# pcannon67/pocketkaldi

Measured on AMD Instinct MI355X. Metric: acoustic frames/sec (fbank->nnet log-likelihoods), higher is better.
Workload: dtype f32

## Files before the change

### pocketkaldi_amd/csrc/capi_batch.hip

```cpp
#include <hip/hip_runtime.h>

#include <algorithm>
#include <mutex>
#include <unordered_set>
#include <vector>

#include "pk_frontend.h"
#include "pk_resample.h"
#include "pk_score.h"

using namespace pkmi;
using namespace pkhost;

namespace pkhost {
struct ArenaRec {
  void *mem;
  bool batch_alive;
  ViewGen *cur;
};
}

namespace {
std::mutex g_arena_mu;
std::unordered_set<const ViewGen *> g_gens;
std::vector<ViewGen *> g_retired;
size_t g_retired_head = 0;

inline unsigned SerialOf(const pk_mi355_am_t *am) { return (unsigned)((reinterpret_cast<uintptr_t>(am) >> 1) & 31u); }
inline pk_mi355_am_t *TagView(ViewGen *g) { return reinterpret_cast<pk_mi355_am_t *>(reinterpret_cast<uintptr_t>(g) | (uintptr_t(g->serial) << 1) | 1u); }
ViewGen *NewGenRecord(pk_mi355_am_t *am, ArenaRec *a, int views) {
  ViewGen *v;
  if (g_retired.size() - g_retired_head >= 64) {
    v = g_retired[g_retired_head++];
    if (g_retired_head > 4096) { g_retired.erase(g_retired.begin(), g_retired.begin() + g_retired_head); g_retired_head = 0; }
  } else {
    v = new ViewGen();
    v->serial = 0;
  }
  v->am = am; v->arena = a; v->live = views; v->current = true; v->withheld = false;
  g_gens.insert(v);
  return v;
}
void RetireGenRecord(ViewGen *v) {
  g_gens.erase(v);
  v->serial = (v->serial + 1) & 31u;
  g_retired.push_back(v);
}
ArenaRec *RegisterArena(void *p) { return new ArenaRec{p, true, nullptr}; }
pk_mi355_am_t *NewViewGen(ArenaRec *a, pk_mi355_am_t *am, int views) {
  std::lock_guard<std::mutex> g(g_arena_mu);
  if (a->cur) {
    a->cur->current = false;
    if (a->cur->live <= 0) RetireGenRecord(a->cur);
  }
  a->cur = NewGenRecord(am, a, views);
  return TagView(a->cur);
}
void RetireArena(ArenaRec *a) {
  void *release = nullptr;
  {
    std::lock_guard<std::mutex> g(g_arena_mu);
    a->batch_alive = false;
    if (!a->cur || a->cur->live <= 0) {
      if (a->cur) RetireGenRecord(a->cur);
      release = a->mem;
      delete a;
    }
  }
  if (release) hipHostFree(release);
}
}

namespace pkhost {
void ReleaseArenaView(pk_mi355_am_t *handle) {
  void *release = nullptr;
  {
    std::lock_guard<std::mutex> g(g_arena_mu);
    ViewGen *v = GenOf(handle);
    if (!g_gens.count(v) || v->serial != SerialOf(handle)) return;
    if (--v->live > 0) return;
    if (v->current) {
      ArenaRec *a = v->arena;
      if (a->batch_alive) return;
      release = a->mem;
      delete a;
    }
    RetireGenRecord(v);
  }
  if (release) hipHostFree(release);
}
}

namespace {
hipStream_t ResultStream(int device) {
  static hipStream_t streams[64] = {};
  if (device < 0 || device >= 64) { Fail(PK_MI355_E_INVALID, "device index %d", device); return nullptr; }
  std::lock_guard<std::mutex> g(g_arena_mu);
  if (!streams[device]) {
    hipError_t e = hipStreamCreateWithFlags(&streams[device], hipStreamNonBlocking);
    if (e != hipSuccess) { Fail(PK_MI355_E_DEVICE, "result stream: %s", hipGetErrorString(e)); return nullptr; }
  }
  return streams[device];
}
}


struct pk_mi355_batch {
  ScorerCore core;
  Timer timer;
  int max_utts = 0;
  int64_t max_samples = 0;
  float *d_wave = nullptr;
  int16_t *d_wave_i16 = nullptr;
  const float *wave_f32 = nullptr;
  const int16_t *wave_i16 = nullptr;
  enum Source { kNone, kWaves, kRaw, kNormalized };
  Source source = kNone;
  bool features_only = false;
  bool have_stats = false;
  FrontendAnyTables *d_any = nullptr;
  float *d_feats = nullptr;
  const float *feats = nullptr;
  Resampler resampler;
  float *h_native = nullptr, *d_native = nullptr;
  int64_t native_cap = 0;
  int num_utts = 0;
  int max_T = 0;
  int64_t total_frames = 0, total_cols = 0;
  int64_t dirty_cols = 0;
  char *h_lay = nullptr, *d_lay = nullptr;
  hipEvent_t ev_layout = nullptr;
  int64_t *h_wave_off = nullptr, *h_raw_base = nullptr, *h_pad_base = nullptr;
  int32_t *h_T = nullptr;
  UttLayout lay{};
  std::vector<int64_t> h_out_base;
  int64_t total_rows = 0;
  bool compact = false;
  const int32_t *d_shift4 = nullptr;
  float *d_raw_alloc = nullptr;
  float *d_raw = nullptr;
  _Float16 *d_y2 = nullptr;
  float *h_ll = nullptr;
  ArenaRec *arena = nullptr;
  hipEvent_t ev_scored = nullptr, ev_fetched = nullptr;
  int lanes = 1;
  hipStream_t stream2 = nullptr;
  ExecBufs exec2;
  hipEvent_t ev_front = nullptr, ev_lane2 = nullptr;
  bool scored = false;
  bool range_pending = false;
  int range_status = 0;
  char range_msg[512] = "";
};

namespace {

constexpr size_t kLayoutEntry = 3 * sizeof(int64_t) + sizeof(int32_t);

int FramesFit(const pk_mi355_batch *b, const int *frames, int num_utts) {
  const int pad = b->core.am->left + b->core.am->right;
  int64_t raw = 0, col = 0;
  for (int u = 0; u < num_utts; ++u) {
    raw += frames[u];
    col += frames[u] > 0 ? frames[u] + pad : 0;
  }
  if (raw > b->core.max_frames || RoundUp(col, kTile) > b->core.max_cols)
    return Fail(PK_MI355_E_INVALID, "frame capacity exceeded (%lld frames, %lld columns; the batch holds %lld and %lld)", (long long)raw,
                (long long)RoundUp(col, kTile), (long long)b->core.max_frames, (long long)b->core.max_cols);
  return 0;
}

int SetLayoutFrames(pk_mi355_batch *b, const int *frames, const int *num_samples, int num_utts) {
  if (int rc = FramesFit(b, frames, num_utts)) return rc;
  ScorerCore &c = b->core;
  const int pad = c.am->left + c.am->right;
  HIP_TRY(hipEventSynchronize(b->ev_layout));
  const size_t n = (size_t)num_utts;
  size_t bytes = kLayoutEntry * n;
  b->h_wave_off = reinterpret_cast<int64_t *>(b->h_lay); b->h_raw_base = b->h_wave_off + n; b->h_pad_base = b->h_raw_base + n;
  b->h_T = reinterpret_cast<int32_t *>(b->h_pad_base + n);
  const int64_t *d64 = reinterpret_cast<const int64_t *>(b->d_lay);
  b->lay = UttLayout{d64, reinterpret_cast<const int32_t *>(d64 + 3 * n), d64 + n, d64 + 2 * n};
  int64_t woff = 0, raw = 0, col = 0;
  b->max_T = 0;
  for (int u = 0; u < num_utts; ++u) {
    const int T = frames[u];
    b->h_wave_off[u] = woff; b->h_raw_base[u] = raw; b->h_pad_base[u] = col; b->h_T[u] = T;
    woff += num_samples ? num_samples[u] : 0;
    raw += T;
    col += T > 0 ? T + pad : 0;
    b->max_T = std::max(b->max_T, T);
  }
  if (col < b->dirty_cols)
    HIP_TRY(hipMemset2DAsync(c.d_yt + col, sizeof(float) * c.ldy, 0, sizeof(float) * (size_t)(b->dirty_cols - col), c.am->feat_dim, c.stream));
  b->dirty_cols = col;
  b->num_utts = num_utts;
  b->total_frames = raw;
  b->total_cols = col;
  b->scored = false;
  b->h_out_base.resize(num_utts);
  b->total_rows = 0;
  int64_t row = 0;
  std::vector<ShiftSpan> spans;
  bool shifted = false;
  for (int u = 0; u < num_utts; ++u) {
    const int T = b->h_T[u];
    b->h_out_base[u] = b->compact ? row : b->h_pad_base[u];
    if (T == 0) continue;
    b->total_rows = b->h_out_base[u] + T;
    row += RoundUp(T, 4);
    spans.push_back({row, (int32_t)(b->h_pad_base[u] - b->h_out_base[u])});
    shifted = shifted || spans.back().shift != 0;
  }
  b->d_shift4 = nullptr;
  if (num_utts == 0) return 0;
  if (shifted) {
    bytes = RoundUp(bytes, 256);
    if (!ExpandShift4(spans, b->total_rows, c.zero_span, reinterpret_cast<int32_t *>(b->h_lay + bytes), nullptr))
      return Fail(PK_MI355_E_INVALID, "internal: column shift outside [0, %lld]", (long long)(c.zero_span - kTile));
    b->d_shift4 = reinterpret_cast<const int32_t *>(b->d_lay + bytes);
    bytes += sizeof(int32_t) * Shift4Groups(b->total_rows);
  }
  HIP_TRY(hipMemcpyAsync(b->d_lay, b->h_lay, bytes, hipMemcpyHostToDevice, c.stream));
  HIP_TRY(hipEventRecord(b->ev_layout, c.stream));
  return 0;
}

int SetLayout(pk_mi355_batch *b, const int *num_samples, int num_utts) {
  if (num_utts < 0 || num_utts > b->max_utts) return Fail(PK_MI355_E_INVALID, "too many utterances (%d > %d)", num_utts, b->max_utts);
  std::vector<int> frames(num_utts);
  int64_t total = 0;
  for (int u = 0; u < num_utts; ++u) {
    if (num_samples[u] < 0) return Fail(PK_MI355_E_INVALID, "negative sample count");
    frames[u] = pk_mi355_num_frames(num_samples[u]);
    total += num_samples[u];
  }
  if (total > b->max_samples) return Fail(PK_MI355_E_INVALID, "too many samples (%lld > %lld)", (long long)total, (long long)b->max_samples);
  if (int rc = SetLayoutFrames(b, frames.data(), num_samples, num_utts)) return rc;
  b->source = pk_mi355_batch::kWaves;
  return 0;
}

int CheckFeatureKind(const pk_mi355_batch *b, int kind) {
  if (kind != PK_MI355_FEATS_NORMALIZED && kind != PK_MI355_FEATS_RAW) return Fail(PK_MI355_E_INVALID, "unknown feature kind %d", kind);
  if (kind == PK_MI355_FEATS_RAW && !b->have_stats) {
    if (b->core.am->feat_dim == kNumBins)
      return Fail(PK_MI355_E_INVALID, "raw features need the CMVN statistics and a %d-dim model (this batch: no statistics, %d-dim)", kNumBins,
                  kNumBins);
    return Fail(PK_MI355_E_INVALID, "raw features need the CMVN statistics: this %d-dim batch was made without them "
                "(pk_mi355_features_batch_create_stats takes the %d of a %d-dim model)", b->core.am->feat_dim, b->core.am->feat_dim + 1,
                b->core.am->feat_dim);
  }
  return 0;
}
int CheckFeatureCounts(const pk_mi355_batch *b, const int *frames, int num_utts) {
  if (num_utts < 0 || num_utts > b->max_utts) return Fail(PK_MI355_E_INVALID, "too many utterances (%d > %d)", num_utts, b->max_utts);
  for (int u = 0; u < num_utts; ++u)
    if (frames[u] < 0) return Fail(PK_MI355_E_INVALID, "utterance %d has a negative frame count (%d)", u, frames[u]);
  return FramesFit(b, frames, num_utts);
}
int EnsureFeatsStaging(pk_mi355_batch *b) {
  if (b->d_feats) return 0;
  HIP_TRY(hipMalloc(&b->d_feats, sizeof(float) * (size_t)b->core.max_frames * b->core.am->feat_dim));
  return 0;
}
int WaveEntryAllowed(const pk_mi355_batch *b) {
  if (b->features_only) return Fail(PK_MI355_E_STATE, "this batch was made by pk_mi355_features_batch_create: it takes features, not audio");
  return 0;
}

int BatchRangeStatus(pk_mi355_batch *b) {
  if (b->range_pending) {
    const ExecBufs *eb[2] = {&b->core.exec, &b->exec2};
    b->range_status = EvalRange(b->core.am, eb, b->lanes == 2 ? 2 : 1);
    if (b->range_status) {
      snprintf(b->range_msg, sizeof(b->range_msg), "%s", LastError());
      std::lock_guard<std::mutex> g(g_arena_mu);
      if (b->arena && b->arena->cur) b->arena->cur->withheld = true;
    }
    b->range_pending = false;
  }
  if (b->range_status) return Fail(b->range_status, "%s", b->range_msg);
  return 0;
}

int64_t TotalSamples(const int *num_samples, int n) {
  int64_t s = 0;
  for (int i = 0; i < n; ++i) s += num_samples[i];
  return s;
}

}

namespace pkhost {
bool BatchScored(const pk_mi355_batch *b) { return b->scored; }
const pk_mi355_am *BatchModel(const pk_mi355_batch *b) { return b->core.am; }

void CreateScorerCore(ScorerCore *c, pk_mi355_am *am, const float *global_stats, int stats_dim, int units, int64_t max_frames,
                      int64_t max_rows, int64_t chunk_cap, CreateCheck &chk) {
  const int pad = am->left + am->right;
  c->am = am; c->device = am->device; c->max_frames = max_frames;
  c->max_cols = RoundUp(max_rows + (int64_t)units * pad, kTileF16);
  c->chunk = std::min<int64_t>(chunk_cap, c->max_cols);
  c->zero_span = ZeroSpan(units, pad);
  c->ldy = RoundUp(c->max_cols, c->chunk) + 256 + c->zero_span;
  auto table = [&](auto **d, const void *h, size_t bytes) {
    chk(hipMalloc(d, bytes));
    if (chk.ok) chk(hipMemcpy(*d, h, bytes, hipMemcpyHostToDevice));
  };
  chk(hipStreamCreate(&c->stream));
  if (global_stats) {
    if (stats_dim == kNumBins) {
      FrontendTables host;
      if (BuildFrontendTables(&host)) { chk.ok = false; Fail(PK_MI355_E_INVALID, "front-end table construction failed"); }
      table(&c->d_tables, &host, sizeof(FrontendTables));
    }
    CmvnTables ctab;
    BuildCmvnTables(global_stats[stats_dim], &ctab);
    table(&c->d_global, global_stats, sizeof(float) * (stats_dim + 1));
    table(&c->d_cmvn_tab, &ctab, sizeof(CmvnTables));
  }
  chk(hipMalloc(&c->d_yt, sizeof(float) * c->ldy * am->feat_dim));
  if (chk.ok) chk(hipMemset(c->d_yt, 0, sizeof(float) * c->ldy * am->feat_dim));
  chk(hipMalloc(&c->d_ll, sizeof(float) * c->max_cols * am->num_pdfs));
  if (chk.ok && AllocExec(am, c->chunk, &c->exec)) chk.ok = false;
}

void FreeScorerCore(ScorerCore *c) {
  FreeExec(&c->exec);
  hipFree(c->d_tables); hipFree(c->d_global); hipFree(c->d_cmvn_tab); hipFree(c->d_yt); hipFree(c->d_ll);
  if (c->stream) hipStreamDestroy(c->stream);
}

bool ExpandShift4(const std::vector<ShiftSpan> &spans, int64_t total_rows, int64_t zero_span, int32_t *shift4, int32_t *bad) {
  int32_t shift = 0;
  int64_t g = 0;
  for (const ShiftSpan &sp : spans) {
    shift = sp.shift;
    if (shift < 0 || shift + kTile > zero_span) { if (bad) *bad = shift; return false; }
    for (; g < sp.end_row / 4; ++g) shift4[g] = shift;
  }
  for (const int64_t groups = Shift4Groups(total_rows); g < groups; ++g) shift4[g] = shift;
  return true;
}
}

extern "C" {

int pk_mi355_num_frames(int num_samples) {
  if (num_samples < kFrameLength) return 0;
  return 1 + (num_samples - kFrameLength) / kFrameShift;
}

}

namespace {
int64_t PublicChunkCap() {
  const char *e = getenv("PK_MI355_CHUNK");
  return e && atol(e) >= kTile ? RoundUp(atol(e), kTileF16) : 262144;
}

pk_mi355_batch *CreateBatch(pk_mi355_am_t *am, const float *global_stats, int max_utts, int64_t max_total_samples, int64_t max_frames,
                            int64_t chunk_cap, const FrontendAnyTables *any = nullptr) {
  if (UseDevice(am->device)) return nullptr;
  pk_mi355_batch *b = new pk_mi355_batch();
  ScorerCore &c = b->core;
  b->max_utts = max_utts; b->max_samples = max_total_samples;
  b->features_only = max_total_samples == 0;
  b->have_stats = global_stats != nullptr;
  const int pad = am->left + am->right;
  CreateCheck chk{b->features_only ? "batch_create_features" : "batch_create"};
  CreateScorerCore(&c, am, global_stats, am->feat_dim, max_utts, max_frames, max_frames, chunk_cap, chk);
  b->compact = pad >= 3;
  if (const char *e = getenv("PK_MI355_COMPACT_ROWS")) b->compact = b->compact && atoi(e) != 0;
  const size_t lay_bytes = RoundUp(kLayoutEntry * max_utts, 256) + (b->compact ? sizeof(int32_t) * Shift4Cap(c.max_cols) : 0);
  chk(hipHostMalloc(reinterpret_cast<void **>(&b->h_lay), lay_bytes, hipHostMallocDefault));
  chk(hipMalloc(&b->d_lay, lay_bytes));
  chk(hipEventCreateWithFlags(&b->ev_layout, hipEventDisableTiming));
  if (b->have_stats && am->feat_dim != kNumBins) {
    chk(hipMalloc(&b->d_raw_alloc, sizeof(float) * (size_t)c.max_frames * am->feat_dim));
    b->d_raw = b->d_raw_alloc;
  } else if (b->have_stats) {
    const size_t raw_floats = (size_t)c.max_frames * kNumBins + kCmvnRawLead + kCmvnRawSlack;
    chk(hipMalloc(&b->d_raw_alloc, sizeof(float) * raw_floats));
    if (chk.ok) chk(hipMemset(b->d_raw_alloc, 0, sizeof(float) * raw_floats));
    if (chk.ok) b->d_raw = b->d_raw_alloc + kCmvnRawLead;
  }
  if (any) {
    if (!c.d_tables && chk.ok) {
      FrontendTables host;
      if (BuildFrontendTables(&host)) { chk.ok = false; Fail(PK_MI355_E_INVALID, "front-end table construction failed"); }
      chk(hipMalloc(&c.d_tables, sizeof(FrontendTables)));
      if (chk.ok) chk(hipMemcpy(c.d_tables, &host, sizeof(FrontendTables), hipMemcpyHostToDevice));
    }
    chk(hipMalloc(&b->d_any, sizeof(FrontendAnyTables)));
    if (chk.ok) chk(hipMemcpy(b->d_any, any, sizeof(FrontendAnyTables), hipMemcpyHostToDevice));
    if (am->feat_dim != kNumBins)
      chk(hipMalloc(&b->d_feats, sizeof(float) * (size_t)c.max_frames * am->feat_dim));
  }
  if (IsF16(am->precision)) chk(hipMalloc(&b->d_y2, sizeof(_Float16) * 2 * c.ldy * am->feat_dim));
  if (const char *e = getenv("PK_MI355_LANES")) b->lanes = atoi(e) >= 2 ? 2 : 1;
  if (c.max_cols <= c.chunk) b->lanes = 1;
  if (b->lanes == 2) {
    chk(hipStreamCreate(&b->stream2));
    chk(hipEventCreateWithFlags(&b->ev_front, hipEventDisableTiming));
    chk(hipEventCreateWithFlags(&b->ev_lane2, hipEventDisableTiming));
    if (chk.ok && AllocExec(am, c.chunk, &b->exec2)) chk.ok = false;
  }
  if (!chk.ok) { pk_mi355_batch_destroy(b); return nullptr; }
  return b;
}

template <class Make>
pk_mi355_batch *EnsureOwned(OwnedBatch *o, int64_t need, bool keep, Make make) {
  if (o->b && need <= o->cap && keep) return o->b;
  if (o->b) pk_mi355_batch_destroy(o->b);
  o->cap = std::max<int64_t>(need, 2 * o->cap);
  o->b = make(o->cap);
  if (!o->b) o->cap = 0;
  return o->b;
}
}

namespace pkhost {
pk_mi355_batch *SingleBatch(pk_mi355_am *am, int64_t frames) {
  return EnsureOwned(&am->single, std::max(frames, kSingleChunk), true,
                     [&](int64_t cap) { return CreateBatch(am, nullptr, 1, 0, cap, kSingleChunk); });
}
}

extern "C" {

pk_mi355_batch_t *pk_mi355_batch_create(pk_mi355_am_t *am, const float *global_stats41, int max_utts, int64_t max_total_samples) {
  if (!am || !am->finalized) { Fail(PK_MI355_E_STATE, "model not finalized"); return nullptr; }
  if (am->feat_dim != kNumBins) { Fail(PK_MI355_E_INVALID, "the front-end produces %d-dim features, the model expects %d", kNumBins, am->feat_dim); return nullptr; }
  if (!global_stats41 || max_utts <= 0 || max_total_samples <= 0) { Fail(PK_MI355_E_INVALID, "bad batch capacity"); return nullptr; }
  return CreateBatch(am, global_stats41, max_utts, max_total_samples, max_total_samples / kFrameShift + max_utts, PublicChunkCap());
}

pk_mi355_batch_t *pk_mi355_features_batch_create(pk_mi355_am_t *am, const float *global_stats41, int max_utts, int64_t max_total_frames) {
  if (!am || !am->finalized) { Fail(PK_MI355_E_STATE, "model not finalized"); return nullptr; }
  if (max_utts <= 0 || max_total_frames <= 0) { Fail(PK_MI355_E_INVALID, "bad batch capacity"); return nullptr; }
  if (global_stats41 && am->feat_dim != kNumBins) {
    Fail(PK_MI355_E_INVALID, "the CMVN statistics are for %d-dim features, the model expects %d", kNumBins, am->feat_dim);
    return nullptr;
  }
  if (IsF16(am->precision) && am->feat_dim % 8 != 0) {
    Fail(PK_MI355_E_INVALID, "f16x3 / f16 precision needs a feature dimension that is a multiple of 8 (got %d)", am->feat_dim);
    return nullptr;
  }
  return CreateBatch(am, global_stats41, max_utts, 0, max_total_frames, PublicChunkCap());
}

pk_mi355_batch_t *pk_mi355_features_batch_create_stats(pk_mi355_am_t *am, const float *global_stats, int stats_len, int max_utts,
                                                       int64_t max_total_frames) {
  if (!am || !am->finalized) { Fail(PK_MI355_E_STATE, "model not finalized"); return nullptr; }
  if (!global_stats) { Fail(PK_MI355_E_INVALID, "null argument"); return nullptr; }
  if (stats_len != am->feat_dim + 1) {
    Fail(PK_MI355_E_INVALID, "the CMVN statistics have %d entries, a %d-dim model needs %d (the sums, then the count)", stats_len, am->feat_dim,
         am->feat_dim + 1);
    return nullptr;
  }
  if (am->feat_dim == kNumBins) return pk_mi355_features_batch_create(am, global_stats, max_utts, max_total_frames);
  if (max_utts <= 0 || max_total_frames <= 0) { Fail(PK_MI355_E_INVALID, "bad batch capacity"); return nullptr; }
  if (IsF16(am->precision) && am->feat_dim % 8 != 0) {
    Fail(PK_MI355_E_INVALID, "f16x3 / f16 precision needs a feature dimension that is a multiple of 8 (got %d)", am->feat_dim);
    return nullptr;
  }
  return CreateBatch(am, global_stats, max_utts, 0, max_total_frames, PublicChunkCap());
}

pk_mi355_batch_t *pk_mi355_frontend_batch_create(pk_mi355_am_t *am, const pk_mi355_frontend_spec_t *spec, const float *global_stats,
                                                 int stats_len, int max_utts, int64_t max_total_samples) {
  if (!am || !am->finalized) { Fail(PK_MI355_E_STATE, "model not finalized"); return nullptr; }
  if (!spec || !global_stats) { Fail(PK_MI355_E_INVALID, "null argument"); return nullptr; }
  std::vector<FrontendAnyTables> any(1);
  if (BuildFrontendAnyTables(spec, any.data())) return nullptr;
  if (any[0].dim != am->feat_dim) {
    Fail(PK_MI355_E_INVALID, "the front-end spec produces %d-dim features, the model expects %d", any[0].dim, am->feat_dim);
    return nullptr;
  }
  if (stats_len != am->feat_dim + 1) {
    Fail(PK_MI355_E_INVALID, "the CMVN statistics have %d entries, a %d-dim model needs %d (the sums, then the count)", stats_len, am->feat_dim,
         am->feat_dim + 1);
    return nullptr;
  }
  if (max_utts <= 0 || max_total_samples <= 0) { Fail(PK_MI355_E_INVALID, "bad batch capacity"); return nullptr; }
  if (IsF16(am->precision) && am->feat_dim % 8 != 0) {
    Fail(PK_MI355_E_INVALID, "f16x3 / f16 precision needs a feature dimension that is a multiple of 8 (got %d)", am->feat_dim);
    return nullptr;
  }
  return CreateBatch(am, global_stats, max_utts, max_total_samples, max_total_samples / kFrameShift + max_utts, PublicChunkCap(), any.data());
}

int pk_mi355_features_dim(const pk_mi355_batch_t *b) { return b ? b->core.am->feat_dim : 0; }

void pk_mi355_batch_destroy(pk_mi355_batch_t *b) {
  if (!b) return;
  hipSetDevice(b->core.device);
  if (b->core.stream) hipStreamSynchronize(b->core.stream);
  if (b->stream2) hipStreamSynchronize(b->stream2);
  FreeExec(&b->exec2);
  for (hipEvent_t e : {b->ev_front, b->ev_lane2, b->ev_scored, b->ev_fetched, b->ev_layout}) if (e) hipEventDestroy(e);
  if (b->stream2) hipStreamDestroy(b->stream2);
  hipFree(b->d_wave); hipFree(b->d_wave_i16); hipFree(b->d_raw_alloc); hipFree(b->d_y2); hipFree(b->d_feats); hipFree(b->d_any);
  b->resampler.Free();
  if (b->h_native) hipHostFree(b->h_native);
  hipFree(b->d_native);
  if (b->h_lay) hipHostFree(b->h_lay);
  hipFree(b->d_lay);
  if (b->arena) RetireArena(b->arena);
  FreeScorerCore(&b->core);
  delete b;
}

int pk_mi355_batch_set_waves(pk_mi355_batch_t *b, const pk_vector_t *waves, int num_utts) {
  if (!b || !waves) return Fail(PK_MI355_E_INVALID, "null argument");
  if (int rc = WaveEntryAllowed(b)) return rc;
  if (int rc = UseDevice(b->core.device)) return rc;
  std::vector<int> ns(num_utts);
  for (int u = 0; u < num_utts; ++u) ns[u] = waves[u].dim;
  if (TotalSamples(ns.data(), num_utts) > b->max_samples) return Fail(PK_MI355_E_INVALID, "too many samples");
  if (!b->d_wave) HIP_TRY(hipMalloc(&b->d_wave, sizeof(float) * b->max_samples));
  int64_t off = 0;
  for (int u = 0; u < num_utts; ++u) {
    if (ns[u] > 0)
      HIP_TRY(hipMemcpyAsync(b->d_wave + off, waves[u].data, sizeof(float) * ns[u], hipMemcpyHostToDevice, b->core.stream));
    off += ns[u];
  }
  b->wave_f32 = b->d_wave;
  b->wave_i16 = nullptr;
  return SetLayout(b, ns.data(), num_utts);
}

int pk_mi355_resample_set_waves(pk_mi355_batch_t *b, const pk_vector_t *waves, const int *rates, int num_utts) {
  if (!b || !waves) return Fail(PK_MI355_E_INVALID, "null argument");
  if (int rc = WaveEntryAllowed(b)) return rc;
  bool native = false;
  for (int u = 0; rates && u < num_utts; ++u) native = native || rates[u] != kSampleRate;
  if (!native) return pk_mi355_batch_set_waves(b, waves, num_utts);
  if (num_utts > b->max_utts) return Fail(PK_MI355_E_INVALID, "too many utterances (%d > %d)", num_utts, b->max_utts);
  if (int rc = UseDevice(b->core.device)) return rc;
  std::vector<int> ns(num_utts);
  std::vector<const DeviceResampleTable *> tab(num_utts, nullptr);
  int64_t total_native = 0;
  for (int u = 0; u < num_utts; ++u) {
    if (waves[u].dim < 0) return Fail(PK_MI355_E_INVALID, "negative sample count");
    if (rates[u] == kSampleRate) { ns[u] = waves[u].dim; continue; }
    if (int rc = b->resampler.Table(rates[u], &tab[u])) return rc;
    const int64_t n_out = ResampleNumOutput(tab[u]->host, waves[u].dim);
    if (n_out > b->max_samples) return Fail(PK_MI355_E_INVALID, "too many samples");
    ns[u] = (int)n_out;
    total_native += waves[u].dim;
  }
  if (TotalSamples(ns.data(), num_utts) > b->max_samples) return Fail(PK_MI355_E_INVALID, "too many samples");
  if (!b->d_wave) HIP_TRY(hipMalloc(&b->d_wave, sizeof(float) * b->max_samples));
  HIP_TRY(hipStreamSynchronize(b->core.stream));
  if (total_native > b->native_cap) {
    const int64_t cap = std::max<int64_t>(total_native, 2 * b->native_cap);
    if (b->h_native) hipHostFree(b->h_native);
    hipFree(b->d_native);
    b->h_native = nullptr; b->d_native = nullptr; b->native_cap = 0;
    HIP_TRY(hipHostMalloc(reinterpret_cast<void **>(&b->h_native), sizeof(float) * cap, hipHostMallocDefault));
    HIP_TRY(hipMalloc(&b->d_native, sizeof(float) * cap));
    b->native_cap = cap;
  }
  std::vector<ResampleItem> items;
  int64_t off = 0, noff = 0;
  for (int u = 0; u < num_utts; ++u) {
    const int n = waves[u].dim;
    if (!tab[u]) {
      if (n > 0) HIP_TRY(hipMemcpyAsync(b->d_wave + off, waves[u].data, sizeof(float) * n, hipMemcpyHostToDevice, b->core.stream));
    } else {
      if (n > 0) memcpy(b->h_native + noff, waves[u].data, sizeof(float) * n);
      if (ns[u] > 0) items.push_back(Resampler::Item(*tab[u], b->d_native + noff, 0, n, 0, ns[u], b->d_wave + off));
      noff += n;
    }
    off += ns[u];
  }
  if (total_native > 0)
    HIP_TRY(hipMemcpyAsync(b->d_native, b->h_native, sizeof(float) * total_native, hipMemcpyHostToDevice, b->core.stream));
  if (int rc = b->resampler.Run(items, b->core.stream)) return rc;
  b->wave_f32 = b->d_wave;
  b->wave_i16 = nullptr;
  return SetLayout(b, ns.data(), num_utts);
}

int pk_mi355_batch_set_waves_i16(pk_mi355_batch_t *b, const int16_t *samples, const int *num_samples,
                                 int num_utts) {
  if (!b || !samples || !num_samples) return Fail(PK_MI355_E_INVALID, "null argument");
  if (int rc = WaveEntryAllowed(b)) return rc;
  if (int rc = UseDevice(b->core.device)) return rc;
  const int64_t total = TotalSamples(num_samples, num_utts);
  if (total > b->max_samples) return Fail(PK_MI355_E_INVALID, "too many samples");
  if (!b->d_wave_i16) HIP_TRY(hipMalloc(&b->d_wave_i16, sizeof(int16_t) * b->max_samples));
  if (total > 0)
    HIP_TRY(hipMemcpyAsync(b->d_wave_i16, samples, sizeof(int16_t) * total, hipMemcpyHostToDevice, b->core.stream));
  b->wave_i16 = b->d_wave_i16;
  b->wave_f32 = nullptr;
  return SetLayout(b, num_samples, num_utts);
}

int pk_mi355_batch_set_waves_device(pk_mi355_batch_t *b, const float *d_samples, const int *num_samples,
                                    int num_utts) {
  if (!b || !d_samples || !num_samples) return Fail(PK_MI355_E_INVALID, "null argument");
  if (int rc = WaveEntryAllowed(b)) return rc;
  if (int rc = UseDevice(b->core.device)) return rc;
  b->wave_f32 = d_samples;
  b->wave_i16 = nullptr;
  return SetLayout(b, num_samples, num_utts);
}

int pk_mi355_features_set(pk_mi355_batch_t *b, const pk_matrix_t *feats, int num_utts, int kind) {
  if (!b || (num_utts > 0 && !feats)) return Fail(PK_MI355_E_INVALID, "null argument");
  if (int rc = CheckFeatureKind(b, kind)) return rc;
  const int D = b->core.am->feat_dim;
  std::vector<int> frames(std::max(num_utts, 0));
  for (int u = 0; u < num_utts; ++u) {
    if (feats[u].nrow != D) return Fail(PK_MI355_E_INVALID, "features of utterance %d have %d rows, the model expects %d", u, feats[u].nrow, D);
    if (feats[u].ncol > 0 && !feats[u].data) return Fail(PK_MI355_E_INVALID, "features of utterance %d: null data", u);
    frames[u] = feats[u].ncol;
  }
  if (int rc = CheckFeatureCounts(b, frames.data(), num_utts)) return rc;
  if (int rc = UseDevice(b->core.device)) return rc;
  float *dst = b->d_raw;
  if (kind == PK_MI355_FEATS_NORMALIZED || D != kNumBins)
    if (int rc = EnsureFeatsStaging(b)) return rc;
  if (kind == PK_MI355_FEATS_NORMALIZED) dst = b->d_feats;
  if (int rc = SetLayoutFrames(b, frames.data(), nullptr, num_utts)) return rc;
  b->source = pk_mi355_batch::kNone;
  int64_t row = 0;
  for (int u = 0; u < num_utts; ++u) {
    if (frames[u] > 0)
      HIP_TRY(hipMemcpyAsync(dst + row * D, feats[u].data, sizeof(float) * (size_t)frames[u] * D, hipMemcpyHostToDevice, b->core.stream));
    row += frames[u];
  }
  if (kind == PK_MI355_FEATS_NORMALIZED) b->feats = b->d_feats;
  b->source = kind == PK_MI355_FEATS_RAW ? pk_mi355_batch::kRaw : pk_mi355_batch::kNormalized;
  return 0;
}

int pk_mi355_features_set_device(pk_mi355_batch_t *b, const float *d_feats, const int *num_frames, int num_utts, int kind) {
  if (!b || (num_utts > 0 && (!d_feats || !num_frames))) return Fail(PK_MI355_E_INVALID, "null argument");
  if (int rc = CheckFeatureKind(b, kind)) return rc;
  if (int rc = CheckFeatureCounts(b, num_frames, num_utts)) return rc;
  if (int rc = UseDevice(b->core.device)) return rc;
  if (kind == PK_MI355_FEATS_RAW) {
    const int D = b->core.am->feat_dim;
    if (D != kNumBins)
      if (int rc = EnsureFeatsStaging(b)) return rc;
    int64_t total = 0;
    for (int u = 0; u < num_utts; ++u) total += num_frames[u];
    if (total > 0)
      HIP_TRY(hipMemcpyAsync(b->d_raw, d_feats, sizeof(float) * (size_t)total * D, hipMemcpyDeviceToDevice, b->core.stream));
  }
  if (int rc = SetLayoutFrames(b, num_frames, nullptr, num_utts)) return rc;
  if (kind == PK_MI355_FEATS_NORMALIZED) b->feats = d_feats;
  b->source = kind == PK_MI355_FEATS_RAW ? pk_mi355_batch::kRaw : pk_mi355_batch::kNormalized;
  return 0;
}

int pk_mi355_batch_score(pk_mi355_batch_t *b, float prob_scale, int sync) {
  if (!b) return Fail(PK_MI355_E_INVALID, "null batch");
  if (b->source == pk_mi355_batch::kNone) return Fail(PK_MI355_E_STATE, "no waves or features set");
  ScorerCore &c = b->core;
  int rc = UseDevice(c.device);
  if (rc) return rc;
  pk_mi355_am *am = c.am;
  Timer *tm = b->timer.enabled ? &b->timer : nullptr;
  if (tm) tm->Reset();
  b->range_pending = false;
  b->range_status = 0;
  b->range_msg[0] = 0;
  b->scored = false;
  if (b->num_utts == 0 || b->total_frames == 0) { b->scored = true; return 0; }
  const UttLayout &lay = b->lay;
  const int D = am->feat_dim;
  if (b->source == pk_mi355_batch::kWaves) {
    Scoped t(tm, PK_MI355_K_FBANK, c.stream);
    if (b->d_any) LaunchFbankAny(b->wave_f32, b->wave_i16, lay, b->num_utts, b->max_T, c.d_tables, b->d_any, D, b->d_raw, c.stream);
    else LaunchFbank(b->wave_f32, b->wave_i16, lay, b->num_utts, b->max_T, c.d_tables, b->d_raw, c.stream);
  }
  {
    Scoped t(tm, PK_MI355_K_CMVN, c.stream);
    if (b->source == pk_mi355_batch::kNormalized)
      LaunchFeatureLayout(b->feats, lay, b->num_utts, b->max_T, D, am->left, am->right, c.d_yt, c.ldy, c.stream);
    else if (D != kNumBins) {
      LaunchCmvnChain(b->d_raw, lay, b->num_utts, D, c.d_global, c.d_cmvn_tab, b->d_feats, c.stream);
      LaunchFeatureLayout(b->d_feats, lay, b->num_utts, b->max_T, D, am->left, am->right, c.d_yt, c.ldy, c.stream);
    } else
      LaunchCmvn(b->d_raw, lay, b->num_utts, c.d_global, c.d_cmvn_tab, am->left, am->right, c.d_yt, c.ldy, c.stream);
  }
  const bool f16 = IsF16(am->precision);
  if (f16) {
    if ((rc = BeginRange(c.exec, c.stream))) return rc;
    Scoped t(tm, PK_MI355_K_OTHER, c.stream);
    const int split_rows = (int)std::min<int64_t>(c.ldy, RoundUp(b->total_cols, kTileF16) + 2 * kTileF16);
    LaunchSplitF16(c.d_yt, 1, c.ldy, split_rows, D, D, b->d_y2, 2 * D, ExpX(am, 0), RangeOf(c.exec, 0), c.stream);
  }
  const bool two = b->lanes == 2 && b->total_rows > c.chunk;
  if (f16 && b->lanes == 2 && !two) ClearHostRange(b->exec2);
  if (two) {
    HIP_TRY(hipEventRecord(b->ev_front, c.stream));
    HIP_TRY(hipStreamWaitEvent(b->stream2, b->ev_front, 0));
    if (f16 && (rc = BeginRange(b->exec2, b->stream2))) return rc;
  }
  const Operand op{c.d_yt, b->d_y2, c.ldy, ZeroSource(c), b->d_shift4};
  const Lane lanes[2] = {{c.stream, &c.exec}, {b->stream2, &b->exec2}};
  if ((rc = WalkChunks(am, op, b->total_rows, c.chunk, lanes, two ? 2 : 1, true, prob_scale, c.d_ll, tm))) return rc;
  if (two) {
    if (f16 && (rc = CollectRange(b->exec2, b->stream2))) return rc;
    HIP_TRY(hipEventRecord(b->ev_lane2, b->stream2));
    HIP_TRY(hipStreamWaitEvent(c.stream, b->ev_lane2, 0));
  }
  if (f16) {
    if ((rc = CollectRange(c.exec, c.stream))) return rc;
    b->range_pending = true;
    b->range_status = 0;
  }
  b->scored = true;
  if (sync) return pk_mi355_batch_synchronize(b);
  return 0;
}

int pk_mi355_batch_synchronize(pk_mi355_batch_t *b) {
  if (!b) return Fail(PK_MI355_E_INVALID, "null batch");
  HIP_TRY(hipStreamSynchronize(b->core.stream));
  return BatchRangeStatus(b);
}

int pk_mi355_batch_calibrate(pk_mi355_batch_t *b) {
  if (!b) return Fail(PK_MI355_E_INVALID, "null batch");
  pk_mi355_am *am = b->core.am;
  if (!IsF16(am->precision)) return 0;
  if (b->source == pk_mi355_batch::kNone) return Fail(PK_MI355_E_STATE, "no waves or features set");
  if (b->total_frames == 0) return Fail(PK_MI355_E_INVALID, "calibration needs at least one frame");
  if (int rc = UseDevice(b->core.device)) return rc;
  std::lock_guard<std::mutex> lock(am->mu);
  return BatchCalibrateLocked(b);
}

}

int pkhost::BatchCalibrateLocked(pk_mi355_batch *b) {
  pk_mi355_am *am = b->core.am;
  if (am->exps_stale) if (int rc = RefreshExps(am)) return rc;
  const ExecBufs &e = b->core.exec;
  return CalibrateLoop(am, e, [&]() -> int {
    const int rc = pk_mi355_batch_score(b, 1.0f, 0);
    b->scored = false;
    b->range_pending = false;
    if (rc) return rc;
    HIP_TRY(hipStreamSynchronize(b->core.stream));
    if (b->lanes == 2)
      for (int i = 0; i < e.range_words; ++i) e.h_range[i] = std::max(e.h_range[i], b->exec2.h_range[i]);
    return 0;
  });
}

extern "C" {

int pk_mi355_batch_num_utts(const pk_mi355_batch_t *b) { return b ? b->num_utts : 0; }
int pk_mi355_batch_num_frames(const pk_mi355_batch_t *b, int utt) {
  return (b && utt >= 0 && utt < b->num_utts) ? b->h_T[utt] : 0;
}
int64_t pk_mi355_batch_total_frames(const pk_mi355_batch_t *b) { return b ? b->total_frames : 0; }

const float *pk_mi355_batch_loglik_device(const pk_mi355_batch_t *b, int utt) {
  if (!b || utt < 0 || utt >= b->num_utts) return nullptr;
  return b->core.d_ll + b->h_out_base[utt] * b->core.am->num_pdfs;
}

int pk_mi355_batch_fetch(pk_mi355_batch_t *b, int utt, pk_decodable_t *out) {
  if (!b || !out || utt < 0 || utt >= b->num_utts) return Fail(PK_MI355_E_INVALID, "bad utterance index");
  if (!b->scored) return Fail(PK_MI355_E_STATE, "batch not scored");
  if (int rc = UseDevice(b->core.device)) return rc;
  ClearDecodable(out, b->core.am);
  if (b->h_T[utt] == 0) return 0;
  return FetchRows(pk_mi355_batch_loglik_device(b, utt), b->h_T[utt], b->core.am->num_pdfs, b->core.stream, "fetch", out,
                   [&] { return BatchRangeStatus(b); });
}

int pk_mi355_batch_fetch_all(pk_mi355_batch_t *b, pk_decodable_t *out, int num_out, int sync) {
  if (!b || !out || num_out != b->num_utts) return Fail(PK_MI355_E_INVALID, "fetch_all: expected %d decodables", b ? b->num_utts : 0);
  if (!b->scored) return Fail(PK_MI355_E_STATE, "batch not scored");
  int rc = UseDevice(b->core.device);
  if (rc) return rc;
  const int N = b->core.am->num_pdfs;
  if (!b->h_ll) {
    const size_t bytes = sizeof(float) * (size_t)b->core.max_cols * N;
    HIP_TRY(hipHostMalloc(reinterpret_cast<void **>(&b->h_ll), bytes, hipHostMallocDefault));
    b->arena = RegisterArena(b->h_ll);
  }
  if (b->total_rows > 0) {
    hipStream_t rs = ResultStream(b->core.device);
    if (!rs) return PK_MI355_E_DEVICE;
    if (!b->ev_scored) {
      HIP_TRY(hipEventCreateWithFlags(&b->ev_scored, hipEventDisableTiming));
      HIP_TRY(hipEventCreateWithFlags(&b->ev_fetched, hipEventDisableTiming));
    }
    HIP_TRY(hipEventRecord(b->ev_scored, b->core.stream));
    HIP_TRY(hipStreamWaitEvent(rs, b->ev_scored, 0));
    HIP_TRY(hipMemcpyAsync(b->h_ll, b->core.d_ll, sizeof(float) * (size_t)b->total_rows * N, hipMemcpyDeviceToHost, rs));
    HIP_TRY(hipEventRecord(b->ev_fetched, rs));
    HIP_TRY(hipStreamWaitEvent(b->core.stream, b->ev_fetched, 0));
  }
  pk_mi355_am_t *gen = NewViewGen(b->arena, b->core.am, num_out);
  for (int u = 0; u < num_out; ++u) {
    const int T = b->h_T[u];
    out[u].am = gen;
    out[u].log_prob.ncol = T;
    out[u].log_prob.nrow = T > 0 ? N : 0;
    out[u].log_prob.data = T > 0 ? b->h_ll + (size_t)b->h_out_base[u] * N : nullptr;
  }
  if (sync && (rc = pk_mi355_batch_synchronize(b))) {
    for (int u = 0; u < num_out; ++u) {
      ReleaseArenaView(gen);
      ClearDecodable(&out[u], b->core.am);
    }
    return rc;
  }
  return 0;
}

int pk_mi355_batch_fetch_fbank(pk_mi355_batch_t *b, int utt, float *out) {
  if (!b || !out || utt < 0 || utt >= b->num_utts) return Fail(PK_MI355_E_INVALID, "bad utterance index");
  if (!b->scored) return Fail(PK_MI355_E_STATE, "batch not scored");
  if (b->source == pk_mi355_batch::kNormalized) return Fail(PK_MI355_E_STATE, "the batch was fed normalised features: there is no fbank");
  const int T = b->h_T[utt];
  if (T == 0) return 0;
  const int D = b->core.am->feat_dim;
  HIP_TRY(hipMemcpyAsync(out, b->d_raw + b->h_raw_base[utt] * D, sizeof(float) * (size_t)T * D, hipMemcpyDeviceToHost, b->core.stream));
  HIP_TRY(hipStreamSynchronize(b->core.stream));
  return 0;
}

int pk_mi355_batch_fetch_cmvn(pk_mi355_batch_t *b, int utt, float *out) {
  if (!b || !out || utt < 0 || utt >= b->num_utts) return Fail(PK_MI355_E_INVALID, "bad utterance index");
  if (!b->scored) return Fail(PK_MI355_E_STATE, "batch not scored");
  const int T = b->h_T[utt];
  if (T == 0) return 0;
  const int D = b->core.am->feat_dim;
  std::vector<float> tmp((size_t)D * T);
  HIP_TRY(hipMemcpy2DAsync(tmp.data(), sizeof(float) * T, b->core.d_yt + b->h_pad_base[utt] + b->core.am->left,
                           sizeof(float) * b->core.ldy, sizeof(float) * T, D, hipMemcpyDeviceToHost, b->core.stream));
  HIP_TRY(hipStreamSynchronize(b->core.stream));
  for (int t = 0; t < T; ++t)
    for (int d = 0; d < D; ++d) out[(size_t)t * D + d] = tmp[(size_t)d * T + t];
  return 0;
}

int pk_mi355_batch_gather_loglik(pk_mi355_batch_t *b, int utt, const int32_t *d_frames,
                                 const int32_t *d_trans_ids, int n, float *d_out) {
  if (!b || utt < 0 || utt >= b->num_utts || !d_frames || !d_trans_ids || !d_out)
    return Fail(PK_MI355_E_INVALID, "bad gather arguments");
  if (!b->scored) return Fail(PK_MI355_E_STATE, "batch not scored");
  if (int rc = UseDevice(b->core.device)) return rc;
  LaunchGather(pk_mi355_batch_loglik_device(b, utt), b->core.am->num_pdfs, b->core.am->d_tid2pdf,
               (int)b->core.am->tid2pdf.size(), d_frames, d_trans_ids, n, d_out, b->core.stream);
  hipError_t e = hipGetLastError();
  if (e != hipSuccess) return Fail(PK_MI355_E_DEVICE, "gather: %s", hipGetErrorString(e));
  return 0;
}

void *pk_mi355_batch_stream(pk_mi355_batch_t *b) { return b ? (void *)b->core.stream : nullptr; }

int pk_mi355_batch_enable_timing(pk_mi355_batch_t *b, int enable) {
  if (!b) return Fail(PK_MI355_E_INVALID, "null batch");
  b->timer.enabled = enable != 0;
  if (!enable) b->timer.Reset();
  return 0;
}

int pk_mi355_batch_get_timing(pk_mi355_batch_t *b, float ms[PK_MI355_K_COUNT], int launches[PK_MI355_K_COUNT]) {
  if (!b) return Fail(PK_MI355_E_INVALID, "null batch");
  for (int k = 0; k < PK_MI355_K_COUNT; ++k) { ms[k] = 0; launches[k] = 0; }
  HIP_TRY(hipStreamSynchronize(b->core.stream));
  for (auto &r : b->timer.recs) {
    float t = 0;
    HIP_TRY(hipEventElapsedTime(&t, r.a, r.b));
    ms[r.kind] += t;
    launches[r.kind] += 1;
  }
  return 0;
}

int pk_mi355_process_acoustic(pk_mi355_am_t *am, const pk_vector_t *cmvn_global_stats,
                              const pk_vector_t *raw_wave, float prob_scale, pk_decodable_t *out,
                              int verbose) {
  if (!am || !cmvn_global_stats || !raw_wave || !out) return Fail(PK_MI355_E_INVALID, "null argument");
  if (cmvn_global_stats->dim != kNumBins + 1) return Fail(PK_MI355_E_INVALID, "cmvn_global_stats must have 41 entries");
  ClearDecodable(out, am);
  if (raw_wave->dim == 0) return 0;
  std::lock_guard<std::mutex> lock(am->mu);
  const float *stats = cmvn_global_stats->data;
  pk_mi355_batch *b = EnsureOwned(&am->proc, std::max<int64_t>(raw_wave->dim, 16000), memcmp(am->proc_stats, stats, sizeof(am->proc_stats)) == 0,
                                  [&](int64_t cap) { return pk_mi355_batch_create(am, stats, 1, cap); });
  if (!b) return PK_MI355_E_DEVICE;
  memcpy(am->proc_stats, stats, sizeof(am->proc_stats));
  int rc = pk_mi355_batch_set_waves(b, raw_wave, 1);
  if (rc) return rc;
  pk_mi355_batch_enable_timing(b, verbose);
  if ((rc = pk_mi355_batch_score(b, prob_scale, 1))) return rc;
  if (verbose) {
    float ms[PK_MI355_K_COUNT];
    int launches[PK_MI355_K_COUNT];
    if ((rc = pk_mi355_batch_get_timing(b, ms, launches))) return rc;
    fprintf(stderr, "Fbank: %lfms\n", (double)ms[PK_MI355_K_FBANK]);
    fprintf(stderr, "CMVN: %lfms\n", (double)ms[PK_MI355_K_CMVN]);
    fprintf(stderr, "NNET: %lfms\n", (double)(ms[PK_MI355_K_GEMM] + ms[PK_MI355_K_TAIL] + ms[PK_MI355_K_OTHER]));
  }
  return pk_mi355_batch_fetch(b, 0, out);
}

}
```

### pocketkaldi_amd/csrc/capi_exec.hip

```cpp
#include <hip/hip_runtime.h>
#include <math.h>

#include <algorithm>
#include <mutex>
#include <vector>

#include "pk_score.h"

using namespace pkmi;
using namespace pkhost;

namespace pkhost {

struct ExecResult { const float *data = nullptr; int64_t ld = 0; int dim = 0; };

int AllocExec(const pk_mi355_am *am, int64_t rows_cap, ExecBufs *e) {
  e->rows_cap = rows_cap;
  if (IsF16(am->precision)) {
    const size_t act = sizeof(_Float16) * 2 * (size_t)am->max_dim_pad * rows_cap;
    const size_t xin = sizeof(_Float16) * 2 * (size_t)RoundUp(am->input_dim, kBKF16) * (rows_cap + 16);
    for (int i = 0; i < 2; ++i) {
      HIP_TRY(hipMalloc(&e->h[i], act));
      HIP_TRY(hipMemset(e->h[i], 0, act));
    }
    HIP_TRY(hipMalloc(&e->xin, xin));
    HIP_TRY(hipMemset(e->xin, 0, xin));
    e->range_words = (int)am->lin.size() * kRangeSlots;
    HIP_TRY(hipMalloc(&e->range, sizeof(uint32_t) * e->range_words));
    HIP_TRY(hipMemset(e->range, 0, sizeof(uint32_t) * e->range_words));
    HIP_TRY(hipHostMalloc(reinterpret_cast<void **>(&e->h_range), sizeof(uint32_t) * e->range_words, hipHostMallocDefault));
    memset(e->h_range, 0, sizeof(uint32_t) * e->range_words);
  }
  {
    const size_t nd = sizeof(unsigned) * (size_t)(rows_cap / kTile + 2);
    HIP_TRY(hipMalloc(&e->row_done, nd));
    HIP_TRY(hipMemset(e->row_done, 0, nd));
    e->row_done_bytes = nd;
  }
  e->act_floats = (int64_t)am->max_dim_pad * rows_cap;
  e->in_floats = RoundUp(am->input_dim, kBK) * rows_cap;
  HIP_TRY(hipMalloc(&e->a, e->act_floats * sizeof(float)));
  HIP_TRY(hipMalloc(&e->b, e->act_floats * sizeof(float)));
  HIP_TRY(hipMalloc(&e->in, e->in_floats * sizeof(float)));
  HIP_TRY(hipMemset(e->a, 0, e->act_floats * sizeof(float)));
  HIP_TRY(hipMemset(e->b, 0, e->act_floats * sizeof(float)));
  HIP_TRY(hipMemset(e->in, 0, e->in_floats * sizeof(float)));
  return 0;
}

void FreeExec(ExecBufs *e) {
  hipFree(e->a);
  hipFree(e->b);
  hipFree(e->in);
  for (int i = 0; i < 2; ++i) hipFree(e->h[i]);
  hipFree(e->xin);
  hipFree(e->range);
  hipFree(e->row_done);
  if (e->h_range) hipHostFree(e->h_range);
  *e = ExecBufs();
}

int BeginRange(const ExecBufs &e, hipStream_t s) {
  if (e.range) HIP_TRY(hipMemsetAsync(e.range, 0, sizeof(uint32_t) * e.range_words, s));
  return 0;
}
int CollectRange(const ExecBufs &e, hipStream_t s) {
  if (e.range) HIP_TRY(hipMemcpyAsync(e.h_range, e.range, sizeof(uint32_t) * e.range_words, hipMemcpyDeviceToHost, s));
  return 0;
}
void ClearHostRange(const ExecBufs &e) {
  if (e.h_range) memset(e.h_range, 0, sizeof(uint32_t) * e.range_words);
}
float RangeMax(const ExecBufs &e, int l) {
  uint32_t m = 0;
  for (int i = 0; i < kRangeSlots; ++i) m = std::max(m, e.h_range[(size_t)l * kRangeSlots + i]);
  float f;
  memcpy(&f, &m, sizeof(f));
  return f;
}
int EvalRange(const pk_mi355_am *am, const ExecBufs *const *bufs, int nbufs) {
  const int nlin = (int)am->lin.size();
  for (int l = 0; l < nlin; ++l) {
    float m = 0.0f;
    for (int i = 0; i < nbufs; ++i)
      if (bufs[i]->h_range) m = std::max(m, RangeMax(*bufs[i], l));
    const int xe = am->exps_stale ? 0 : am->h_exps[nlin + l];
    const char *mode = am->precision == PK_MI355_PRECISION_F16 ? "f16" : "f16x3";
    if (m >= kRangeSaturated)
      return Fail(PK_MI355_E_RANGE, "%s range: the input of affine layer %d saturated (|x| * 2^%d reached 65504, the fp16 split "
                  "clamps there): results withheld; lower the operand's exponent (pk_mi355_am_calibrate)", mode, l, xe);
    if (m > 0.0f && m < kRangeTooSmall)
      return Fail(PK_MI355_E_RANGE, "%s range: the input of affine layer %d is too small for the fp16 split (max |x| * 2^%d = %g "
                  "< 2^-5: every low half is subnormal): results withheld; raise the operand's exponent "
                  "(pk_mi355_am_calibrate)", mode, l, xe, (double)m);
  }
  return 0;
}


int RunLayers(const pk_mi355_am *am, const ExecBufs &e, const float *q0, int64_t ldq,
              int splice_dim, int rows, bool want_tail, float scale, float *tail_out,
              int64_t tail_ld, hipStream_t stream, Timer *timer, ExecResult *res, const float *splice_zero = nullptr,
              const int32_t *splice_shift = nullptr) {
  const int rows_pad = (int)RoundUp(rows, kTile);
  if (splice_dim > 0 && !splice_zero) return Fail(PK_MI355_E_INVALID, "spliced input without a zero source");
  if (rows_pad > e.rows_cap) return Fail(PK_MI355_E_INVALID, "chunk larger than workspace");
  const float *blob = am->d_blob;
  const int nl = (int)am->layers.size();

  int last_linear = -1;
  for (int i = 0; i < nl; ++i)
    if (am->layers[i].type == PK_NNET_LINEAR_LAYER) last_linear = i;

  const float *cur = splice_dim > 0 ? q0 : e.in;
  int64_t cur_ld = splice_dim > 0 ? ldq : e.rows_cap;
  bool cur_rows = false;
  bool cur_splice = splice_dim > 0;
  int cur_dim = am->input_dim;
  float *bufs[2] = {e.a, e.b};
  int next_buf = 0;
  int li_lin = 0;
  bool tail_done = false;

  auto to_rows = [&]() {
    float *dst = bufs[next_buf];
    const int64_t ld = RoundUp(cur_dim, kTile);
    Scoped t(timer, PK_MI355_K_OTHER, stream);
    LaunchTransposeToRows(cur, cur_ld, cur_dim, rows_pad, dst, ld, stream);
    cur = dst; cur_ld = ld; cur_rows = true; next_buf ^= 1;
  };

  for (int i = 0; i < nl; ++i) {
    const HostLayer &L = am->layers[i];
    switch (L.type) {
      case PK_NNET_LINEAR_LAYER: {
        const DevLinear &D = am->lin[li_lin++];
        if (cur_rows) return Fail(PK_MI355_E_INVALID, "linear layer after a softmax is not supported");
        const bool fuse_relu = (i + 1 < nl && am->layers[i + 1].type == PK_NNET_RELU_LAYER);
        const bool rows_out = (i == last_linear) && !cur_splice;
        float *dst = bufs[next_buf];
        GemmArgs g;
        g.K = D.Kpad;
        g.relu = fuse_relu ? 1 : 0;
        g.bias = blob + D.b_off;
        g.out = dst;
        if (!rows_out) {
          g.P = blob + D.wt_off; g.ldp = D.Npad;
          g.Q = cur; g.ldq = cur_ld;
          g.splice_dim = cur_splice ? splice_dim : 0;
          if (cur_splice) {
            g.splice_ctx = am->left + am->right + 1;
            g.splice_zero = splice_zero;
            g.splice_shift = splice_shift;
            g.ring = am->knobs.l1_ring;
          }
          g.bias_on_j = 0;
          g.ldo = e.rows_cap;
          g.tiles_i = D.Npad / kTile; g.tiles_j = rows_pad / kTile;
        } else {
          g.P = cur; g.ldp = cur_ld;
          g.Q = blob + D.wt_off; g.ldq = D.Npad;
          g.splice_dim = 0;
          g.bias_on_j = 1;
          g.ldo = D.Npad;
          g.tiles_i = rows_pad / kTile; g.tiles_j = D.Npad / kTile;
        }
        bool fused_tail = false;
        if (rows_out && want_tail && !fuse_relu && !am->softmax_reference && i + 2 == nl &&
            am->layers[i + 1].type == PK_NNET_SOFTMAX_LAYER && am->knobs.wave_tail32) {
          g.tail_out = tail_out; g.tail_ld = tail_ld;
          g.tail_log_prior = blob + am->logprior_off; g.tail_scale = scale;
          g.tail_n = D.N; g.tail_rows = rows; g.row_done = e.row_done;
          g.tail_walk = am->knobs.tail_walk;
          fused_tail = GemmFusesTail(g, am->knobs.fused_tail_min_tiles);
          if (!fused_tail) g.tail_out = nullptr;
          else HIP_TRY(hipMemsetAsync(e.row_done, 0, sizeof(unsigned) * (size_t)g.tiles_i, stream));
        }
        {
          Scoped t(timer, PK_MI355_K_GEMM, stream);
          GemmArgs fewer = g;
          fewer.tiles_j -= 1;
          if (fused_tail && am->knobs.tail_strip && g.tiles_j > 8 && D.N <= (g.tiles_j - 1) * kTile + kTile / 2 &&
              GemmFusesTail(fewer, am->knobs.fused_tail_min_tiles)) {
            GemmArgs s = g;
            const int j0 = (g.tiles_j - 1) * kTile;
            s.Q = g.Q + j0; s.bias = g.bias + j0; s.out = g.out + j0;
            s.half_j = 1;
            s.tail_out = nullptr;
            LaunchGemm(s, stream);
            g.tiles_j -= 1;
          }
          LaunchGemm(g, stream);
        }
        cur = dst; cur_ld = g.ldo; cur_rows = rows_out; cur_splice = false; cur_dim = D.N;
        next_buf ^= 1;
        if (fuse_relu) ++i;
        if (fused_tail) { tail_done = true; ++i; }
        break;
      }
      case PK_NNET_RELU_LAYER: {
        if (cur_splice || cur == e.in) {
          float *dst = bufs[next_buf];
          if (cur_splice) return Fail(PK_MI355_E_INVALID, "network must start with a linear layer when splicing");
          HIP_TRY(hipMemcpyAsync(dst, cur, sizeof(float) * (size_t)RoundUp(cur_dim, kBK) * e.rows_cap,
                                 hipMemcpyDeviceToDevice, stream));
          cur = dst; next_buf ^= 1;
        }
        Scoped t(timer, PK_MI355_K_OTHER, stream);
        const int64_t n = cur_rows ? (int64_t)rows_pad * cur_ld : (int64_t)cur_dim * cur_ld;
        LaunchRelu(const_cast<float *>(cur), n, stream);
        break;
      }
      case PK_NNET_NORMALIZE_LAYER: {
        if (cur_splice) return Fail(PK_MI355_E_INVALID, "network must start with a linear layer when splicing");
        if (cur == e.in) {
          float *dst = bufs[next_buf];
          HIP_TRY(hipMemcpyAsync(dst, cur, sizeof(float) * (size_t)RoundUp(cur_dim, kBK) * e.rows_cap,
                                 hipMemcpyDeviceToDevice, stream));
          cur = dst; next_buf ^= 1;
        }
        Scoped t(timer, PK_MI355_K_OTHER, stream);
        if (cur_rows) LaunchNormalize(const_cast<float *>(cur), rows_pad, cur_dim, cur_ld, 1, stream);
        else LaunchNormalize(const_cast<float *>(cur), rows_pad, cur_dim, 1, cur_ld, stream);
        break;
      }
      case PK_NNET_SOFTMAX_LAYER: {
        if (cur_splice) return Fail(PK_MI355_E_INVALID, "network must start with a linear layer when splicing");
        if (!cur_rows) to_rows();
        const bool final_layer = (i == nl - 1);
        Scoped t(timer, PK_MI355_K_TAIL, stream);
        if (final_layer && want_tail) {
          if (!(am->knobs.wave_tail32 && !am->softmax_reference &&
                LaunchTailWave(cur, cur_ld, rows, cur_dim, blob + am->logprior_off, scale, tail_out, tail_ld, stream)))
            LaunchTail(kTailSoftmaxLoglik, am->softmax_reference, cur, cur_ld, rows, cur_dim,
                       blob + am->logprior_off, scale, tail_out, tail_ld, stream);
          tail_done = true;
        } else {
          float *dst = bufs[next_buf];
          const int64_t ld = RoundUp(cur_dim, kTile);
          LaunchTail(kTailSoftmaxProb, am->softmax_reference, cur, cur_ld, rows_pad, cur_dim, nullptr, 1.0f, dst, ld, stream);
          cur = dst; cur_ld = ld; next_buf ^= 1;
        }
        break;
      }
      default:
        return Fail(PK_MI355_E_INVALID, "unknown layer type %d", L.type);
    }
  }
  if (!cur_rows && !tail_done) {
    if (cur_splice) return Fail(PK_MI355_E_INVALID, "empty network");
    to_rows();
  }
  if (want_tail && !tail_done) {
    Scoped t(timer, PK_MI355_K_TAIL, stream);
    LaunchTail(kTailLoglik, am->softmax_reference, cur, cur_ld, rows, cur_dim, blob + am->logprior_off,
               scale, tail_out, tail_ld, stream);
  }
  if (res) { res->data = cur; res->ld = cur_ld; res->dim = cur_dim; }
  hipError_t le = hipGetLastError();
  if (le != hipSuccess) return Fail(PK_MI355_E_DEVICE, "kernel launch failed: %s", hipGetErrorString(le));
  return 0;
}

int RunLayersF16(const pk_mi355_am *am, const ExecBufs &e, const _Float16 *x, int64_t ldx, int rows,
                 bool want_tail, float scale, float *tail_out,
                 int64_t tail_ld, hipStream_t stream, Timer *timer, ExecResult *res, const int32_t *row_shift4 = nullptr) {
  const int rows_pad = (int)RoundUp(rows, kTileF16);
  if (rows_pad > e.rows_cap) return Fail(PK_MI355_E_INVALID, "chunk larger than workspace");
  const float *blob = am->d_blob;
  const int nl = (int)am->layers.size();
  const int nlin = (int)am->lin.size();
  int li = 0, buf = 0;
  int64_t out_ld = 0;
  for (int i = 0; i < nl; ++i) {
    if (am->layers[i].type != PK_NNET_LINEAR_LAYER) continue;
    const DevLinear &D = am->lin[li];
    const bool last = (li == nlin - 1);
    GemmF16Args g;
    g.X = x; g.ldx = ldx;
    g.row_shift4 = li == 0 ? row_shift4 : nullptr;
    g.W = reinterpret_cast<const _Float16 *>(blob + D.wt_off);
    g.ldw = 2 * D.Kpad;
    g.K = D.Kpad;
    g.bias = blob + D.b_off;
    g.relu = (i + 1 < nl && am->layers[i + 1].type == PK_NNET_RELU_LAYER) ? 1 : 0;
    const int after = i + 1 + g.relu;
    const bool norm = after < nl && am->layers[after].type == PK_NNET_NORMALIZE_LAYER;
    g.out_f32 = (last || norm) ? e.a : nullptr;
    g.out = (last || norm) ? nullptr : e.h[buf];
    g.ldo = (last || norm) ? D.Npad : 2 * D.Npad;
    g.tiles_m = rows_pad / kTileF16;
    g.tiles_n = D.Npad / kTileF16;
    g.terms = am->precision == PK_MI355_PRECISION_F16 ? 1 : 3;
    g.e_w = ExpW(am, li);
    g.e_in = ExpX(am, li);
    g.e_out = (last || norm) ? ExpZero(am) : ExpX(am, li + 1);
    g.range = (last || norm) ? nullptr : RangeOf(e, li + 1);
    {
      Scoped t(timer, PK_MI355_K_GEMM, stream);
      LaunchGemmF16(g, stream);
    }
    if (norm) {
      Scoped t(timer, PK_MI355_K_OTHER, stream);
      LaunchNormalizeSplitF16(e.a, D.Npad, rows_pad, D.N, D.Npad, e.h[buf], 2 * D.Npad, ExpX(am, li + 1), RangeOf(e, li + 1), stream);
    }
    x = e.h[buf]; ldx = 2 * D.Npad;
    out_ld = D.Npad;
    buf ^= 1;
    ++li;
  }
  const int dim = am->output_dim;
  const bool softmax_last = am->layers.back().type == PK_NNET_SOFTMAX_LAYER;
  const float *cur = e.a;
  if (want_tail) {
    Scoped t(timer, PK_MI355_K_TAIL, stream);
    LaunchTail(softmax_last ? kTailSoftmaxLoglik : kTailLoglik, am->softmax_reference, cur, out_ld, rows, dim,
               blob + am->logprior_off, scale, tail_out, tail_ld, stream);
  } else if (softmax_last) {
    Scoped t(timer, PK_MI355_K_TAIL, stream);
    LaunchTail(kTailSoftmaxProb, am->softmax_reference, cur, out_ld, rows_pad, dim, nullptr, 1.0f, e.b, out_ld, stream);
    cur = e.b;
  }
  if (res) { res->data = cur; res->ld = out_ld; res->dim = dim; }
  hipError_t le = hipGetLastError();
  if (le != hipSuccess) return Fail(PK_MI355_E_DEVICE, "kernel launch failed: %s", hipGetErrorString(le));
  return 0;
}

int WalkChunks(const pk_mi355_am *am, const Operand &op, int64_t total_rows, int64_t chunk, const Lane *lanes, int nlanes,
               bool want_tail, float scale, float *out, Timer *timer) {
  const int D = am->feat_dim, N = am->num_pdfs;
  const bool f16 = IsF16(am->precision);
  for (int64_t r0 = 0; r0 < total_rows; r0 += chunk) {
    const int rows = (int)std::min<int64_t>(chunk, total_rows - r0);
    const Lane &l = lanes[r0 / chunk % nlanes];
    const int32_t *shift4 = op.shift4 ? op.shift4 + r0 / 4 : nullptr;
    float *dst = out + r0 * N;
    const int rc = f16 ? RunLayersF16(am, *l.exec, op.y2 + r0 * 2 * D, 2 * D, rows, want_tail, scale, dst, N, l.stream, timer, nullptr, shift4)
                       : RunLayers(am, *l.exec, op.yt + r0, op.ld, D, rows, want_tail, scale, dst, N, l.stream, timer, nullptr, op.zero, shift4);
    if (rc) return rc;
  }
  return 0;
}

struct Workspace {
  ExecBufs exec;
  float *d_feats = nullptr;  int64_t feats_cap = 0;
  hipStream_t stream = nullptr;
};

int EnsureWorkspace(pk_mi355_am *am, int64_t feats_floats) {
  if (!am->ws) {
    am->ws = new Workspace();
    HIP_TRY(hipStreamCreate(&am->ws->stream));
    int rc = AllocExec(am, kSingleChunk, &am->ws->exec);
    if (rc) return rc;
  }
  Workspace *w = am->ws;
  if (feats_floats > w->feats_cap) {
    hipFree(w->d_feats);
    w->feats_cap = feats_floats;
    HIP_TRY(hipMalloc(&w->d_feats, sizeof(float) * w->feats_cap));
  }
  return 0;
}

void FreeWorkspace(Workspace *w) {
  if (!w) return;
  FreeExec(&w->exec);
  hipFree(w->d_feats);
  if (w->stream) hipStreamDestroy(w->stream);
  delete w;
}

int ResizeHostMatrix(pk_matrix_t *m, int nrow, int ncol) {
  const size_t total = (size_t)nrow * ncol;
  float *p = nullptr;
  if (total > 0) {
    p = static_cast<float *>(realloc(m->data, sizeof(float) * total));
    if (!p) return Fail(PK_MI355_E_INVALID, "out of host memory");
  } else {
    free(m->data);
  }
  m->data = p;
  m->nrow = nrow;
  m->ncol = ncol;
  return 0;
}

int CalibrateStep(pk_mi355_am *am, const ExecBufs &e, std::vector<char> *settled) {
  const int nlin = (int)am->lin.size();
  static const int target = [] { const char *t = getenv("PK_MI355_CALIB_TARGET_LOG2"); const int v = t ? atoi(t) : 3; return v >= 0 && v <= 12 ? v : 3; }();
  for (int l = 0; l < nlin; ++l) {
    const float m = RangeMax(e, l);
    int32_t &xe = am->h_exps[nlin + l];
    int want = xe;
    if (m >= kRangeSaturated) want = xe - 12;
    else if (m > 0.0f && (!(*settled)[l] || m < ldexpf(1.0f, target - 2) || m >= ldexpf(1.0f, target + 4))) { want = xe + target - ilogbf(m); (*settled)[l] = 1; }
    else (*settled)[l] = 1;
    want = std::min(kMaxXExp, std::max(-kMaxXExp, want));
    if (want != xe) { xe = want; return 1; }
  }
  return 0;
}

int CalibrateLoop(pk_mi355_am *am, const ExecBufs &e, const std::function<int()> &pass) {
  const int max_passes = 6 * (int)am->lin.size() + 8;
  std::vector<char> settled(am->lin.size(), 0);
  for (int i = 0, rc; i < max_passes; ++i) {
    if ((rc = pass())) return rc;
    if (!CalibrateStep(am, e, &settled)) {
      const ExecBufs *eb = &e;
      return EvalRange(am, &eb, 1);
    }
    if ((rc = UploadExps(am))) return rc;
  }
  return Fail(PK_MI355_E_RANGE, "calibration did not settle in %d passes", max_passes);
}

}

extern "C" {

int pk_mi355_nnet_propagate(pk_mi355_am_t *am, const pk_matrix_t *in, pk_matrix_t *out) {
  if (!am || !am->finalized) return Fail(PK_MI355_E_STATE, "model not finalized");
  if (!in || !out || in->nrow != am->input_dim)
    return Fail(PK_MI355_E_INVALID, "input has %d rows, the network expects %d", in ? in->nrow : -1, am->input_dim);
  int rc = UseDevice(am->device);
  if (rc) return rc;
  std::lock_guard<std::mutex> lock(am->mu);
  const int T = in->ncol, D = in->nrow;
  if ((rc = ResizeHostMatrix(out, am->output_dim, T))) return rc;
  if (T == 0) return 0;
  if ((rc = EnsureWorkspace(am, (int64_t)T * D))) return rc;
  Workspace *w = am->ws;
  HIP_TRY(hipMemcpyAsync(w->d_feats, in->data, sizeof(float) * (size_t)T * D, hipMemcpyHostToDevice, w->stream));
  for (int64_t r0 = 0; r0 < T; r0 += kSingleChunk) {
    const int rows = (int)std::min<int64_t>(kSingleChunk, T - r0);
    ExecResult res;
    if (IsF16(am->precision)) {
      const int kp = (int)RoundUp(D, kBKF16);
      if ((rc = BeginRange(w->exec, w->stream))) return rc;
      const int64_t rows_pad = RoundUp(rows, kTileF16);
      if (rows_pad > rows)
        HIP_TRY(hipMemsetAsync(w->exec.xin + (size_t)rows * 2 * kp, 0, sizeof(_Float16) * 2 * kp * (size_t)(rows_pad - rows), w->stream));
      LaunchSplitF16(w->d_feats + r0 * D, D, 1, rows, D, kp, w->exec.xin, 2 * kp, ExpX(am, 0), RangeOf(w->exec, 0), w->stream);
      rc = RunLayersF16(am, w->exec, w->exec.xin, 2 * kp, rows, false, 1.0f, nullptr, 0, w->stream, nullptr, &res);
      if (!rc) rc = CollectRange(w->exec, w->stream);
    } else {
      LaunchTransposeToCols(w->d_feats + r0 * D, D, rows, D, w->exec.in, w->exec.rows_cap, w->stream);
      rc = RunLayers(am, w->exec, nullptr, 0, 0, rows, false, 1.0f, nullptr, 0, w->stream, nullptr, &res);
    }
    if (rc) return rc;
    HIP_TRY(hipMemcpy2DAsync(out->data + r0 * am->output_dim, sizeof(float) * am->output_dim, res.data,
                             sizeof(float) * res.ld, sizeof(float) * am->output_dim, rows,
                             hipMemcpyDeviceToHost, w->stream));
    HIP_TRY(hipStreamSynchronize(w->stream));
    if (IsF16(am->precision)) {
      const ExecBufs *eb = &w->exec;
      if ((rc = EvalRange(am, &eb, 1))) { ResizeHostMatrix(out, 0, 0); return rc; }
    }
  }
  return 0;
}


void pk_decodable_init(pk_decodable_t *self, pk_mi355_am_t *am, float prob_scale,
                       const pk_matrix_t *feats) {
  ClearDecodable(self, am);
  if (!am || !am->finalized) { Fail(PK_MI355_E_STATE, "model not finalized"); return; }
  if (!feats || feats->nrow != am->feat_dim) {
    Fail(PK_MI355_E_INVALID, "features have %d rows, the model expects %d", feats ? feats->nrow : -1, am->feat_dim);
    return;
  }
  if (UseDevice(am->device)) return;
  const int T = feats->ncol, D = feats->nrow;
  if (T <= 0) return;
  if (IsF16(am->precision) && D % 8 != 0) {
    Fail(PK_MI355_E_INVALID, "f16x3 / f16 precision needs a feature dimension that is a multiple of 8 (got %d)", D);
    return;
  }
  std::lock_guard<std::mutex> lock(am->mu);
  pk_mi355_batch *b = SingleBatch(am, T);
  if (!b || pk_mi355_features_set(b, feats, 1, PK_MI355_FEATS_NORMALIZED) || pk_mi355_batch_score(b, prob_scale, 0)) return;
  pk_mi355_batch_fetch(b, 0, self);
}

void pk_decodable_destroy(pk_decodable_t *self) {
  if (IsView(self->am)) ReleaseArenaView(self->am);
  else free(self->log_prob.data);
  ClearDecodable(self, nullptr);
}

float pk_decodable_loglikelihood(pk_decodable_t *self, int frame, int trans_id) {
  if (IsView(self->am) && GenOf(self->am)->withheld) return NAN;
  const int pdf = pk_mi355_am_transition_to_pdf(Untag(self->am), trans_id);
  return self->log_prob.data[(size_t)frame * self->log_prob.nrow + pdf];
}

bool pk_decodable_islastframe(pk_decodable_t *self, int frame) {
  return frame == self->log_prob.ncol - 1;
}

int pk_mi355_am_calibrate(pk_mi355_am_t *am, const pk_matrix_t *feats) {
  if (!am || !am->finalized) return Fail(PK_MI355_E_STATE, "model not finalized");
  if (!IsF16(am->precision)) return 0;
  if (!feats || feats->nrow != am->feat_dim || feats->ncol <= 0 || !feats->data)
    return Fail(PK_MI355_E_INVALID, "calibration features have %d rows, the model expects %d", feats ? feats->nrow : -1, am->feat_dim);
  if (feats->nrow % 8 != 0) return Fail(PK_MI355_E_INVALID, "f16x3 / f16 precision needs a feature dimension that is a multiple of 8 (got %d)", feats->nrow);
  int rc = UseDevice(am->device);
  if (rc) return rc;
  std::lock_guard<std::mutex> lock(am->mu);
  pk_mi355_batch *b = SingleBatch(am, feats->ncol);
  if (!b) return PK_MI355_E_DEVICE;
  if ((rc = pk_mi355_features_set(b, feats, 1, PK_MI355_FEATS_NORMALIZED))) return rc;
  return BatchCalibrateLocked(b);
}

}
```

### pocketkaldi_amd/csrc/pk_host.h

```cpp
#ifndef PK_HOST_H_
#define PK_HOST_H_

#include <hip/hip_runtime.h>
#include <stdint.h>
#include <stdio.h>
#include <stdlib.h>
#include <string.h>

#include <mutex>
#include <string>
#include <vector>

#include "pk_files.h"
#include "pk_kernels.h"
#include "pk_tables.h"

namespace pkhost {

using namespace pkmi;


int CurrentDevice();
int UseDevice(int device);

#define HIP_TRY(expr)                                                                  \
  do {                                                                                 \
    hipError_t e_ = (expr);                                                            \
    if (e_ != hipSuccess)                                                              \
      return ::pkhost::Fail(PK_MI355_E_DEVICE, "%s failed: %s (%s:%d)", #expr, hipGetErrorString(e_), \
                            __FILE__, __LINE__);                                       \
  } while (0)

inline int64_t RoundUp(int64_t v, int64_t m) { return (v + m - 1) / m * m; }
inline bool IsF16(int precision) { return precision == PK_MI355_PRECISION_F16X3 || precision == PK_MI355_PRECISION_F16; }

struct ModelKnobs {
  bool wave_tail32 = true;
  int fused_tail_min_tiles = 384;
  int tail_walk = 0;
  int l1_ring = 2;
  bool tail_strip = true;
};
ModelKnobs ReadModelKnobs();


struct Timer {
  bool enabled = false;
  struct Rec { int kind; hipEvent_t a, b; };
  std::vector<Rec> recs;
  std::vector<hipEvent_t> pool;
  hipEvent_t Get() {
    if (!pool.empty()) { hipEvent_t e = pool.back(); pool.pop_back(); return e; }
    hipEvent_t e;
    hipEventCreate(&e);
    return e;
  }
  void Reset() {
    for (auto &r : recs) { pool.push_back(r.a); pool.push_back(r.b); }
    recs.clear();
  }
  int Begin(int kind, hipStream_t s) {
    if (!enabled) return -1;
    Rec r{kind, Get(), Get()};
    hipEventRecord(r.a, s);
    recs.push_back(r);
    return (int)recs.size() - 1;
  }
  void End(int id, hipStream_t s) {
    if (id >= 0) hipEventRecord(recs[id].b, s);
  }
  ~Timer() {
    Reset();
    for (auto e : pool) hipEventDestroy(e);
  }
};

struct Scoped {
  Timer *t; int id; hipStream_t s;
  Scoped(Timer *t_, int kind, hipStream_t s_) : t(t_), id(t_ ? t_->Begin(kind, s_) : -1), s(s_) {}
  ~Scoped() { if (t) t->End(id, s); }
};


struct DevLinear {
  int K = 0, N = 0, Kpad = 0, Npad = 0;
  size_t wt_off = 0, b_off = 0;
};

struct Workspace;

struct OwnedBatch { pk_mi355_batch *b = nullptr; int64_t cap = 0; };

}

struct pk_mi355_am {
  int device = 0;
  std::vector<pkhost::HostLayer> layers;
  bool finalized = false;
  int precision = PK_MI355_PRECISION_F32;
  bool softmax_reference = false;
  int left = 0, right = 0, num_pdfs = 0;
  int input_dim = 0, output_dim = 0, feat_dim = 0;
  int max_dim_pad = 0;
  std::vector<int32_t> tid2pdf;
  int32_t *d_tid2pdf = nullptr;
  std::vector<pkhost::DevLinear> lin;
  float *d_blob = nullptr;
  size_t blob_floats = 0;
  size_t logprior_off = 0;
  size_t exp_off = 0;
  std::vector<int32_t> h_exps;
  bool exps_stale = false;
  double flops_per_frame = 0;
  pkhost::ModelKnobs knobs;
  std::mutex mu;
  pkhost::Workspace *ws = nullptr;
  pkhost::OwnedBatch proc;
  pkhost::OwnedBatch single;
  float proc_stats[41] = {0};
};

namespace pkhost {

int RefreshExps(pk_mi355_am *am);
int UploadExps(pk_mi355_am *am);


struct ExecBufs {
  float *in = nullptr;
  float *a = nullptr;
  float *b = nullptr;
  int64_t rows_cap = 0;
  int64_t in_floats = 0, act_floats = 0;
  _Float16 *h[2] = {nullptr, nullptr};
  _Float16 *xin = nullptr;
  uint32_t *range = nullptr, *h_range = nullptr;
  int range_words = 0;
  unsigned *row_done = nullptr;
  size_t row_done_bytes = 0;
};

int AllocExec(const pk_mi355_am *am, int64_t rows_cap, ExecBufs *e);
void FreeExec(ExecBufs *e);

inline const int32_t *ExpBase(const pk_mi355_am *am) { return reinterpret_cast<const int32_t *>(am->d_blob + am->exp_off); }
inline const int32_t *ExpW(const pk_mi355_am *am, int l) { return ExpBase(am) + l; }
inline const int32_t *ExpX(const pk_mi355_am *am, int l) { return ExpBase(am) + am->lin.size() + l; }
inline const int32_t *ExpZero(const pk_mi355_am *am) { return ExpBase(am) + 2 * am->lin.size(); }
inline uint32_t *RangeOf(const ExecBufs &e, int l) { return e.range ? e.range + (size_t)l * kRangeSlots : nullptr; }

constexpr int kMaxXExp = 30;
constexpr float kRangeSaturated = 65504.0f;
constexpr float kRangeTooSmall = 0.03125f;

int BeginRange(const ExecBufs &e, hipStream_t s);
int CollectRange(const ExecBufs &e, hipStream_t s);
void ClearHostRange(const ExecBufs &e);
int EvalRange(const pk_mi355_am *am, const ExecBufs *const *bufs, int nbufs);
void FreeWorkspace(Workspace *w);
int ResizeHostMatrix(pk_matrix_t *m, int nrow, int ncol);


struct ArenaRec;
struct alignas(64) ViewGen {
  pk_mi355_am_t *am;
  ArenaRec *arena;
  int live;
  bool current;
  bool withheld;
  unsigned serial;
};
inline bool IsView(const pk_mi355_am_t *am) { return (reinterpret_cast<uintptr_t>(am) & 1u) != 0; }
inline ViewGen *GenOf(const pk_mi355_am_t *am) { return reinterpret_cast<ViewGen *>(reinterpret_cast<uintptr_t>(am) & ~uintptr_t(63)); }
inline pk_mi355_am_t *Untag(pk_mi355_am_t *am) { return IsView(am) ? GenOf(am)->am : am; }
void ReleaseArenaView(pk_mi355_am_t *handle);

bool BatchScored(const pk_mi355_batch *b);
const pk_mi355_am *BatchModel(const pk_mi355_batch *b);

const pk_mi355_am *StreamModel(const pk_mi355_stream *s);
int StreamSlots(const pk_mi355_stream *s);
hipStream_t StreamHipStream(const pk_mi355_stream *s);
const float *StreamLoglikBase(const pk_mi355_stream *s);
bool StreamSlotFlushed(const pk_mi355_stream *s, int slot);

bool OnlineDecoderSlotOpen(const pk_mi355_online_decoder *o, int slot);
const std::vector<int> *OnlineDecoderCommittedWords(const pk_mi355_online_decoder *o, int slot);
void OnlineDecoderTailWords(const pk_mi355_online_decoder *o, int slot, std::vector<int> *words);

struct RecognizerFiles {
  pk_mi355_fst_t *fst = nullptr;
  pk_mi355_symtab_t *symtab = nullptr;
};
int LoadRecognizerFiles(const char *config_path, RecognizerFiles *out, bool any_stats = false);
constexpr int kMaxCmvnStats = 129;
void FreeRecognizerFiles(RecognizerFiles *f);
int JoinWords(const pk_mi355_symtab_t *symtab, const int *words, int count, std::string *text);

}

#endif
```

### pocketkaldi_amd/csrc/pk_score.h

```cpp
#ifndef PK_SCORE_H_
#define PK_SCORE_H_

#include <functional>

#include "pk_host.h"

namespace pkmi {

constexpr int kTailCap = kFrameLength;

struct StreamRec {
  int32_t slot;
  int32_t tail_len;
  int32_t new_len;
  int32_t tail_par;
  int32_t n_old;
  int32_t m;
  int32_t a, b;
  int32_t closed;
  int32_t cols;
  int32_t kind;
  int32_t hist_par;
  int64_t woff;
  int64_t new_off;
  int64_t raw_base;
  int64_t col_base;
  int64_t row_off;
};

void LaunchStreamAssemble(const StreamRec *recs, int n, const float *upload, float *tails, float *wave, hipStream_t stream);
void LaunchStreamCmvn(const StreamRec *recs, int n, float *rows, const float *g, const CmvnTables *tab, float *sums,
                      float *raw_hist, float *hist, int hist_len, int left, int right, float *yt, int64_t ldy, hipStream_t stream);

void LaunchStreamRawRows(const StreamRec *recs, int n, const float *upload, float *rows, hipStream_t stream);
void LaunchStreamFeatureLayout(const StreamRec *recs, int n, int max_cols, const float *upload, float *hist, int hist_len, int dim,
                               int left, int right, float *yt, int64_t ldy, hipStream_t stream);

void LaunchFeatureLayout(const float *feats, const UttLayout &utts, int num_utts, int max_frames, int dim, int left, int right,
                         float *yt, int64_t ldy, hipStream_t stream);

void LaunchCmvnChain(const float *raw, const UttLayout &utts, int num_utts, int dim, const float *d_global, const CmvnTables *d_cmvn_tab,
                     float *out, hipStream_t stream);
void LaunchStreamCmvnChain(const StreamRec *recs, int n, int dim, float *upload, const float *g, const CmvnTables *tab, float *sums,
                           float *raw_hist, hipStream_t stream);

}

namespace pkhost {

struct ScorerCore {
  pk_mi355_am *am = nullptr; int device = 0; hipStream_t stream = nullptr;
  FrontendTables *d_tables = nullptr; float *d_global = nullptr; CmvnTables *d_cmvn_tab = nullptr;
  int64_t max_frames = 0, max_cols = 0, chunk = 0, zero_span = 0, ldy = 0;
  float *d_yt = nullptr, *d_ll = nullptr;
  ExecBufs exec;
};

inline int64_t ZeroSpan(int64_t units, int pad) { return RoundUp(units * pad + 2 * kTile, 256); }
inline const float *ZeroSource(const float *yt, int64_t ld, int64_t zero_span) { return yt + (ld - zero_span); }
inline const float *ZeroSource(const ScorerCore &c) { return ZeroSource(c.d_yt, c.ldy, c.zero_span); }

struct CreateCheck {
  const char *name; bool ok = true;
  void operator()(hipError_t e) { if (e != hipSuccess && ok) { ok = false; Fail(PK_MI355_E_DEVICE, "%s: %s", name, hipGetErrorString(e)); } }
};
void CreateScorerCore(ScorerCore *c, pk_mi355_am *am, const float *global_stats, int stats_dim, int units, int64_t max_frames,
                      int64_t max_rows, int64_t chunk_cap, CreateCheck &chk);
void FreeScorerCore(ScorerCore *c);

struct ShiftSpan { int64_t end_row; int32_t shift; };
inline int64_t Shift4Groups(int64_t total_rows) { return RoundUp(total_rows, kTileF16) / 4 + kTileF16 / 4; }
inline int64_t Shift4Cap(int64_t max_cols) { return max_cols / 4 + kTileF16; }
bool ExpandShift4(const std::vector<ShiftSpan> &spans, int64_t total_rows, int64_t zero_span, int32_t *shift4, int32_t *bad);

struct Operand { const float *yt; const _Float16 *y2; int64_t ld; const float *zero; const int32_t *shift4; };
struct Lane { hipStream_t stream; const ExecBufs *exec; };
int WalkChunks(const pk_mi355_am *am, const Operand &op, int64_t total_rows, int64_t chunk, const Lane *lanes, int nlanes,
               bool want_tail, float scale, float *out, Timer *timer);

int CalibrateLoop(pk_mi355_am *am, const ExecBufs &e, const std::function<int()> &pass);

constexpr int64_t kSingleChunk = 4096;
pk_mi355_batch *SingleBatch(pk_mi355_am *am, int64_t frames);
int BatchCalibrateLocked(pk_mi355_batch *b);

inline void ClearDecodable(pk_decodable_t *out, pk_mi355_am_t *am) { out->am = am; out->log_prob = pk_matrix_t{0, 0, nullptr}; }
template <class Verdict>
int FetchRows(const float *src, int rows, int N, hipStream_t stream, const char *what, pk_decodable_t *out, Verdict verdict) {
  const size_t bytes = sizeof(float) * (size_t)rows * N;
  float *host = static_cast<float *>(malloc(bytes));
  if (!host) return Fail(PK_MI355_E_INVALID, "out of host memory");
  hipError_t e = hipMemcpyAsync(host, src, bytes, hipMemcpyDeviceToHost, stream);
  if (e == hipSuccess) e = hipStreamSynchronize(stream);
  if (e != hipSuccess) { free(host); return Fail(PK_MI355_E_DEVICE, "%s: %s", what, hipGetErrorString(e)); }
  if (int rc = verdict()) { free(host); return rc; }
  out->log_prob = pk_matrix_t{rows, N, host};
  return 0;
}

}

#endif
```

Baseline: 10.54 million.

## Run input upload and frontend on a separate stream to overlap with scoring

Adds a dedicated input stream per batch that carries the waveform/feature upload, layout copy, fbank, CMVN and f16 split for large batches. Consumption events are recorded after the first layer reads the spliced input, so the next batch's frontend can overlap the previous batch's nnet layers. Range tracking is split per layer so the first layer's range belongs to the input stream. This adds cross-stream event bookkeeping and risks ordering bugs around shared buffers (d_yt, d_raw, layout).

Result: no change. 10.53 million (-0.1%).

```diff
diff --git a/pocketkaldi_amd/csrc/capi_batch.hip b/pocketkaldi_amd/csrc/capi_batch.hip
--- a/pocketkaldi_amd/csrc/capi_batch.hip
+++ b/pocketkaldi_amd/csrc/capi_batch.hip
@@ -146,7 +146,12 @@
   int lanes = 1;
   hipStream_t stream2 = nullptr;
   ExecBufs exec2;
-  hipEvent_t ev_front = nullptr, ev_lane2 = nullptr;
+  hipEvent_t ev_lane_go = nullptr, ev_lane2 = nullptr;
+  int in_mode = 0;
+  int64_t in_min_frames = 0;
+  hipStream_t in_stream = nullptr;
+  hipEvent_t ev_front = nullptr, ev_consumed = nullptr, ev_consumed2 = nullptr, ev_caller = nullptr;
+  bool in_dirty = false, lay_dirty = false, consumed_new = false;
   bool scored = false;
   bool range_pending = false;
   int range_status = 0;
@@ -170,7 +175,61 @@
   return 0;
 }
 
-int SetLayoutFrames(pk_mi355_batch *b, const int *frames, const int *num_samples, int num_utts) {
+bool Pipelined(const pk_mi355_batch *b, int64_t frames, bool timed) { return b->in_stream && !timed && frames >= b->in_min_frames; }
+
+int InputStream(pk_mi355_batch *b, bool pipelined, hipStream_t *s) {
+  ScorerCore &c = b->core;
+  *s = c.stream;
+  if (!b->in_stream) return 0;
+  if (pipelined) {
+    if (b->lay_dirty) {
+      HIP_TRY(hipEventRecord(b->ev_consumed, c.stream));
+      b->lay_dirty = false;
+      b->consumed_new = true;
+    }
+    if (b->consumed_new) {
+      HIP_TRY(hipStreamWaitEvent(b->in_stream, b->ev_consumed, 0));
+      if (b->lanes == 2) HIP_TRY(hipStreamWaitEvent(b->in_stream, b->ev_consumed2, 0));
+      b->consumed_new = false;
+    }
+    b->in_dirty = true;
+    *s = b->in_stream;
+  } else {
+    if (b->in_dirty) {
+      HIP_TRY(hipEventRecord(b->ev_front, b->in_stream));
+      HIP_TRY(hipStreamWaitEvent(c.stream, b->ev_front, 0));
+      b->in_dirty = false;
+    }
+    b->lay_dirty = true;
+  }
+  return 0;
+}
+int SetStream(pk_mi355_batch *b, int64_t frames, hipStream_t *s) { return InputStream(b, Pipelined(b, frames, false), s); }
+int BehindCaller(pk_mi355_batch *b, hipStream_t s) {
+  if (s == b->core.stream) return 0;
+  HIP_TRY(hipEventRecord(b->ev_caller, b->core.stream));
+  HIP_TRY(hipStreamWaitEvent(s, b->ev_caller, 0));
+  return 0;
+}
+int JoinInput(pk_mi355_batch *b) {
+  if (!b->in_dirty) return 0;
+  HIP_TRY(hipEventRecord(b->ev_front, b->in_stream));
+  HIP_TRY(hipStreamWaitEvent(b->core.stream, b->ev_front, 0));
+  b->in_dirty = false;
+  return 0;
+}
+int64_t WaveFrames(const int *num_samples, int n) {
+  int64_t f = 0;
+  for (int i = 0; i < n; ++i) f += pk_mi355_num_frames(num_samples[i]);
+  return f;
+}
+int64_t SumFrames(const int *frames, int n) {
+  int64_t f = 0;
+  for (int i = 0; i < n; ++i) f += frames[i];
+  return f;
+}
+
+int SetLayoutFrames(pk_mi355_batch *b, const int *frames, const int *num_samples, int num_utts, hipStream_t stream) {
   if (int rc = FramesFit(b, frames, num_utts)) return rc;
   ScorerCore &c = b->core;
   const int pad = c.am->left + c.am->right;
@@ -192,7 +251,7 @@
     b->max_T = std::max(b->max_T, T);
   }
   if (col < b->dirty_cols)
-    HIP_TRY(hipMemset2DAsync(c.d_yt + col, sizeof(float) * c.ldy, 0, sizeof(float) * (size_t)(b->dirty_cols - col), c.am->feat_dim, c.stream));
+    HIP_TRY(hipMemset2DAsync(c.d_yt + col, sizeof(float) * c.ldy, 0, sizeof(float) * (size_t)(b->dirty_cols - col), c.am->feat_dim, stream));
   b->dirty_cols = col;
   b->num_utts = num_utts;
   b->total_frames = raw;
@@ -221,12 +280,12 @@
     b->d_shift4 = reinterpret_cast<const int32_t *>(b->d_lay + bytes);
     bytes += sizeof(int32_t) * Shift4Groups(b->total_rows);
   }
-  HIP_TRY(hipMemcpyAsync(b->d_lay, b->h_lay, bytes, hipMemcpyHostToDevice, c.stream));
-  HIP_TRY(hipEventRecord(b->ev_layout, c.stream));
-  return 0;
-}
-
-int SetLayout(pk_mi355_batch *b, const int *num_samples, int num_utts) {
+  HIP_TRY(hipMemcpyAsync(b->d_lay, b->h_lay, bytes, hipMemcpyHostToDevice, stream));
+  HIP_TRY(hipEventRecord(b->ev_layout, stream));
+  return 0;
+}
+
+int SetLayout(pk_mi355_batch *b, const int *num_samples, int num_utts, hipStream_t stream) {
   if (num_utts < 0 || num_utts > b->max_utts) return Fail(PK_MI355_E_INVALID, "too many utterances (%d > %d)", num_utts, b->max_utts);
   std::vector<int> frames(num_utts);
   int64_t total = 0;
@@ -236,7 +295,7 @@
     total += num_samples[u];
   }
   if (total > b->max_samples) return Fail(PK_MI355_E_INVALID, "too many samples (%lld > %lld)", (long long)total, (long long)b->max_samples);
-  if (int rc = SetLayoutFrames(b, frames.data(), num_samples, num_utts)) return rc;
+  if (int rc = SetLayoutFrames(b, frames.data(), num_samples, num_utts, stream)) return rc;
   b->source = pk_mi355_batch::kWaves;
   return 0;
 }
@@ -355,13 +414,16 @@
 }
 
 namespace {
+constexpr int kInputStreamDefault = 1;
+constexpr int64_t kInputStreamMinFrames = 131072;
+
 int64_t PublicChunkCap() {
   const char *e = getenv("PK_MI355_CHUNK");
   return e && atol(e) >= kTile ? RoundUp(atol(e), kTileF16) : 262144;
 }
 
 pk_mi355_batch *CreateBatch(pk_mi355_am_t *am, const float *global_stats, int max_utts, int64_t max_total_samples, int64_t max_frames,
-                            int64_t chunk_cap, const FrontendAnyTables *any = nullptr) {
+                            int64_t chunk_cap, const FrontendAnyTables *any = nullptr, bool input_stream = true) {
   if (UseDevice(am->device)) return nullptr;
   pk_mi355_batch *b = new pk_mi355_batch();
   ScorerCore &c = b->core;
@@ -403,9 +465,20 @@
   if (c.max_cols <= c.chunk) b->lanes = 1;
   if (b->lanes == 2) {
     chk(hipStreamCreate(&b->stream2));
-    chk(hipEventCreateWithFlags(&b->ev_front, hipEventDisableTiming));
+    chk(hipEventCreateWithFlags(&b->ev_lane_go, hipEventDisableTiming));
     chk(hipEventCreateWithFlags(&b->ev_lane2, hipEventDisableTiming));
     if (chk.ok && AllocExec(am, c.chunk, &b->exec2)) chk.ok = false;
+  }
+  b->in_mode = input_stream ? kInputStreamDefault : 0;
+  b->in_min_frames = kInputStreamMinFrames;
+  if (const char *e = getenv("PK_MI355_INPUT_STREAM")) b->in_mode = input_stream ? std::min(std::max(atoi(e), 0), 2) : 0;
+  if (const char *e = getenv("PK_MI355_INPUT_STREAM_MIN_FRAMES")) b->in_min_frames = std::max<int64_t>(atoll(e), 0);
+  if (b->in_mode) {
+    int least = 0, greatest = 0;
+    chk(hipDeviceGetStreamPriorityRange(&least, &greatest));
+    if (b->in_mode == 2) chk(hipStreamCreateWithPriority(&b->in_stream, hipStreamDefault, least));
+    else chk(hipStreamCreate(&b->in_stream));
+    for (hipEvent_t *e : {&b->ev_front, &b->ev_consumed, &b->ev_consumed2, &b->ev_caller}) chk(hipEventCreateWithFlags(e, hipEventDisableTiming));
   }
   if (!chk.ok) { pk_mi355_batch_destroy(b); return nullptr; }
   return b;
@@ -425,7 +498,7 @@
 namespace pkhost {
 pk_mi355_batch *SingleBatch(pk_mi355_am *am, int64_t frames) {
   return EnsureOwned(&am->single, std::max(frames, kSingleChunk), true,
-                     [&](int64_t cap) { return CreateBatch(am, nullptr, 1, 0, cap, kSingleChunk); });
+                     [&](int64_t cap) { return CreateBatch(am, nullptr, 1, 0, cap, kSingleChunk, nullptr, false); });
 }
 }
 
@@ -500,9 +573,12 @@
   hipSetDevice(b->core.device);
   if (b->core.stream) hipStreamSynchronize(b->core.stream);
   if (b->stream2) hipStreamSynchronize(b->stream2);
+  if (b->in_stream) hipStreamSynchronize(b->in_stream);
   FreeExec(&b->exec2);
-  for (hipEvent_t e : {b->ev_front, b->ev_lane2, b->ev_scored, b->ev_fetched, b->ev_layout}) if (e) hipEventDestroy(e);
+  for (hipEvent_t e : {b->ev_lane_go, b->ev_lane2, b->ev_scored, b->ev_fetched, b->ev_layout, b->ev_front, b->ev_consumed, b->ev_consumed2, b->ev_caller})
+    if (e) hipEventDestroy(e);
   if (b->stream2) hipStreamDestroy(b->stream2);
+  if (b->in_stream) hipStreamDestroy(b->in_stream);
   hipFree(b->d_wave); hipFree(b->d_wave_i16); hipFree(b->d_raw_alloc); hipFree(b->d_y2); hipFree(b->d_feats); hipFree(b->d_any);
   b->resampler.Free();
   if (b->h_native) hipHostFree(b->h_native);
@@ -522,15 +598,17 @@
   for (int u = 0; u < num_utts; ++u) ns[u] = waves[u].dim;
   if (TotalSamples(ns.data(), num_utts) > b->max_samples) return Fail(PK_MI355_E_INVALID, "too many samples");
   if (!b->d_wave) HIP_TRY(hipMalloc(&b->d_wave, sizeof(float) * b->max_samples));
+  hipStream_t st;
+  if (int rc = SetStream(b, WaveFrames(ns.data(), num_utts), &st)) return rc;
   int64_t off = 0;
   for (int u = 0; u < num_utts; ++u) {
     if (ns[u] > 0)
-      HIP_TRY(hipMemcpyAsync(b->d_wave + off, waves[u].data, sizeof(float) * ns[u], hipMemcpyHostToDevice, b->core.stream));
+      HIP_TRY(hipMemcpyAsync(b->d_wave + off, waves[u].data, sizeof(float) * ns[u], hipMemcpyHostToDevice, st));
     off += ns[u];
   }
   b->wave_f32 = b->d_wave;
   b->wave_i16 = nullptr;
-  return SetLayout(b, ns.data(), num_utts);
+  return SetLayout(b, ns.data(), num_utts, st);
 }
 
 int pk_mi355_resample_set_waves(pk_mi355_batch_t *b, const pk_vector_t *waves, const int *rates, int num_utts) {
@@ -555,7 +633,9 @@
   }
   if (TotalSamples(ns.data(), num_utts) > b->max_samples) return Fail(PK_MI355_E_INVALID, "too many samples");
   if (!b->d_wave) HIP_TRY(hipMalloc(&b->d_wave, sizeof(float) * b->max_samples));
-  HIP_TRY(hipStreamSynchronize(b->core.stream));
+  hipStream_t st;
+  if (int rc = SetStream(b, WaveFrames(ns.data(), num_utts), &st)) return rc;
+  HIP_TRY(hipStreamSynchronize(st));
   if (total_native > b->native_cap) {
     const int64_t cap = std::max<int64_t>(total_native, 2 * b->native_cap);
     if (b->h_native) hipHostFree(b->h_native);
@@ -570,7 +650,7 @@
   for (int u = 0; u < num_utts; ++u) {
     const int n = waves[u].dim;
     if (!tab[u]) {
-      if (n > 0) HIP_TRY(hipMemcpyAsync(b->d_wave + off, waves[u].data, sizeof(float) * n, hipMemcpyHostToDevice, b->core.stream));
+      if (n > 0) HIP_TRY(hipMemcpyAsync(b->d_wave + off, waves[u].data, sizeof(float) * n, hipMemcpyHostToDevice, st));
     } else {
       if (n > 0) memcpy(b->h_native + noff, waves[u].data, sizeof(float) * n);
       if (ns[u] > 0) items.push_back(Resampler::Item(*tab[u], b->d_native + noff, 0, n, 0, ns[u], b->d_wave + off));
@@ -579,11 +659,11 @@
     off += ns[u];
   }
   if (total_native > 0)
-    HIP_TRY(hipMemcpyAsync(b->d_native, b->h_native, sizeof(float) * total_native, hipMemcpyHostToDevice, b->core.stream));
-  if (int rc = b->resampler.Run(items, b->core.stream)) return rc;
+    HIP_TRY(hipMemcpyAsync(b->d_native, b->h_native, sizeof(float) * total_native, hipMemcpyHostToDevice, st));
+  if (int rc = b->resampler.Run(items, st)) return rc;
   b->wave_f32 = b->d_wave;
   b->wave_i16 = nullptr;
-  return SetLayout(b, ns.data(), num_utts);
+  return SetLayout(b, ns.data(), num_utts, st);
 }
 
 int pk_mi355_batch_set_waves_i16(pk_mi355_batch_t *b, const int16_t *samples, const int *num_samples,
@@ -594,11 +674,13 @@
   const int64_t total = TotalSamples(num_samples, num_utts);
   if (total > b->max_samples) return Fail(PK_MI355_E_INVALID, "too many samples");
   if (!b->d_wave_i16) HIP_TRY(hipMalloc(&b->d_wave_i16, sizeof(int16_t) * b->max_samples));
+  hipStream_t st;
+  if (int rc = SetStream(b, WaveFrames(num_samples, num_utts), &st)) return rc;
   if (total > 0)
-    HIP_TRY(hipMemcpyAsync(b->d_wave_i16, samples, sizeof(int16_t) * total, hipMemcpyHostToDevice, b->core.stream));
+    HIP_TRY(hipMemcpyAsync(b->d_wave_i16, samples, sizeof(int16_t) * total, hipMemcpyHostToDevice, st));
   b->wave_i16 = b->d_wave_i16;
   b->wave_f32 = nullptr;
-  return SetLayout(b, num_samples, num_utts);
+  return SetLayout(b, num_samples, num_utts, st);
 }
 
 int pk_mi355_batch_set_waves_device(pk_mi355_batch_t *b, const float *d_samples, const int *num_samples,
@@ -606,9 +688,12 @@
   if (!b || !d_samples || !num_samples) return Fail(PK_MI355_E_INVALID, "null argument");
   if (int rc = WaveEntryAllowed(b)) return rc;
   if (int rc = UseDevice(b->core.device)) return rc;
+  hipStream_t st;
+  if (int rc = SetStream(b, WaveFrames(num_samples, num_utts), &st)) return rc;
+  if (int rc = BehindCaller(b, st)) return rc;
   b->wave_f32 = d_samples;
   b->wave_i16 = nullptr;
-  return SetLayout(b, num_samples, num_utts);
+  return SetLayout(b, num_samples, num_utts, st);
 }
 
 int pk_mi355_features_set(pk_mi355_batch_t *b, const pk_matrix_t *feats, int num_utts, int kind) {
@@ -627,12 +712,14 @@
   if (kind == PK_MI355_FEATS_NORMALIZED || D != kNumBins)
     if (int rc = EnsureFeatsStaging(b)) return rc;
   if (kind == PK_MI355_FEATS_NORMALIZED) dst = b->d_feats;
-  if (int rc = SetLayoutFrames(b, frames.data(), nullptr, num_utts)) return rc;
+  hipStream_t st;
+  if (int rc = SetStream(b, SumFrames(frames.data(), num_utts), &st)) return rc;
+  if (int rc = SetLayoutFrames(b, frames.data(), nullptr, num_utts, st)) return rc;
   b->source = pk_mi355_batch::kNone;
   int64_t row = 0;
   for (int u = 0; u < num_utts; ++u) {
     if (frames[u] > 0)
-      HIP_TRY(hipMemcpyAsync(dst + row * D, feats[u].data, sizeof(float) * (size_t)frames[u] * D, hipMemcpyHostToDevice, b->core.stream));
+      HIP_TRY(hipMemcpyAsync(dst + row * D, feats[u].data, sizeof(float) * (size_t)frames[u] * D, hipMemcpyHostToDevice, st));
     row += frames[u];
   }
   if (kind == PK_MI355_FEATS_NORMALIZED) b->feats = b->d_feats;
@@ -645,6 +732,9 @@
   if (int rc = CheckFeatureKind(b, kind)) return rc;
   if (int rc = CheckFeatureCounts(b, num_frames, num_utts)) return rc;
   if (int rc = UseDevice(b->core.device)) return rc;
+  hipStream_t st;
+  if (int rc = SetStream(b, SumFrames(num_frames, num_utts), &st)) return rc;
+  if (int rc = BehindCaller(b, st)) return rc;
   if (kind == PK_MI355_FEATS_RAW) {
     const int D = b->core.am->feat_dim;
     if (D != kNumBins)
@@ -652,9 +742,9 @@
     int64_t total = 0;
     for (int u = 0; u < num_utts; ++u) total += num_frames[u];
     if (total > 0)
-      HIP_TRY(hipMemcpyAsync(b->d_raw, d_feats, sizeof(float) * (size_t)total * D, hipMemcpyDeviceToDevice, b->core.stream));
-  }
-  if (int rc = SetLayoutFrames(b, num_frames, nullptr, num_utts)) return rc;
+      HIP_TRY(hipMemcpyAsync(b->d_raw, d_feats, sizeof(float) * (size_t)total * D, hipMemcpyDeviceToDevice, st));
+  }
+  if (int rc = SetLayoutFrames(b, num_frames, nullptr, num_utts, st)) return rc;
   if (kind == PK_MI355_FEATS_NORMALIZED) b->feats = d_feats;
   b->source = kind == PK_MI355_FEATS_RAW ? pk_mi355_batch::kRaw : pk_mi355_batch::kNormalized;
   return 0;
@@ -676,45 +766,53 @@
   if (b->num_utts == 0 || b->total_frames == 0) { b->scored = true; return 0; }
   const UttLayout &lay = b->lay;
   const int D = am->feat_dim;
+  const bool pipelined = Pipelined(b, b->total_frames, tm != nullptr);
+  hipStream_t fs;
+  if ((rc = InputStream(b, pipelined, &fs))) return rc;
   if (b->source == pk_mi355_batch::kWaves) {
-    Scoped t(tm, PK_MI355_K_FBANK, c.stream);
-    if (b->d_any) LaunchFbankAny(b->wave_f32, b->wave_i16, lay, b->num_utts, b->max_T, c.d_tables, b->d_any, D, b->d_raw, c.stream);
-    else LaunchFbank(b->wave_f32, b->wave_i16, lay, b->num_utts, b->max_T, c.d_tables, b->d_raw, c.stream);
+    Scoped t(tm, PK_MI355_K_FBANK, fs);
+    if (b->d_any) LaunchFbankAny(b->wave_f32, b->wave_i16, lay, b->num_utts, b->max_T, c.d_tables, b->d_any, D, b->d_raw, fs);
+    else LaunchFbank(b->wave_f32, b->wave_i16, lay, b->num_utts, b->max_T, c.d_tables, b->d_raw, fs);
   }
   {
-    Scoped t(tm, PK_MI355_K_CMVN, c.stream);
+    Scoped t(tm, PK_MI355_K_CMVN, fs);
     if (b->source == pk_mi355_batch::kNormalized)
-      LaunchFeatureLayout(b->feats, lay, b->num_utts, b->max_T, D, am->left, am->right, c.d_yt, c.ldy, c.stream);
+      LaunchFeatureLayout(b->feats, lay, b->num_utts, b->max_T, D, am->left, am->right, c.d_yt, c.ldy, fs);
     else if (D != kNumBins) {
-      LaunchCmvnChain(b->d_raw, lay, b->num_utts, D, c.d_global, c.d_cmvn_tab, b->d_feats, c.stream);
-      LaunchFeatureLayout(b->d_feats, lay, b->num_utts, b->max_T, D, am->left, am->right, c.d_yt, c.ldy, c.stream);
+      LaunchCmvnChain(b->d_raw, lay, b->num_utts, D, c.d_global, c.d_cmvn_tab, b->d_feats, fs);
+      LaunchFeatureLayout(b->d_feats, lay, b->num_utts, b->max_T, D, am->left, am->right, c.d_yt, c.ldy, fs);
     } else
-      LaunchCmvn(b->d_raw, lay, b->num_utts, c.d_global, c.d_cmvn_tab, am->left, am->right, c.d_yt, c.ldy, c.stream);
+      LaunchCmvn(b->d_raw, lay, b->num_utts, c.d_global, c.d_cmvn_tab, am->left, am->right, c.d_yt, c.ldy, fs);
   }
   const bool f16 = IsF16(am->precision);
+  const int first_own = f16 && b->in_stream ? 1 : 0;
   if (f16) {
-    if ((rc = BeginRange(c.exec, c.stream))) return rc;
-    Scoped t(tm, PK_MI355_K_OTHER, c.stream);
+    if ((rc = first_own ? BeginRange(c.exec, fs, 0, 1) : BeginRange(c.exec, c.stream))) return rc;
+    Scoped t(tm, PK_MI355_K_OTHER, fs);
     const int split_rows = (int)std::min<int64_t>(c.ldy, RoundUp(b->total_cols, kTileF16) + 2 * kTileF16);
-    LaunchSplitF16(c.d_yt, 1, c.ldy, split_rows, D, D, b->d_y2, 2 * D, ExpX(am, 0), RangeOf(c.exec, 0), c.stream);
-  }
+    LaunchSplitF16(c.d_yt, 1, c.ldy, split_rows, D, D, b->d_y2, 2 * D, ExpX(am, 0), RangeOf(c.exec, 0), fs);
+  }
+  if (first_own && (rc = CollectRange(c.exec, fs, 0, 1))) return rc;
+  if (pipelined && (rc = JoinInput(b))) return rc;
+  if (first_own && (rc = BeginRange(c.exec, c.stream, 1))) return rc;
   const bool two = b->lanes == 2 && b->total_rows > c.chunk;
   if (f16 && b->lanes == 2 && !two) ClearHostRange(b->exec2);
   if (two) {
-    HIP_TRY(hipEventRecord(b->ev_front, c.stream));
-    HIP_TRY(hipStreamWaitEvent(b->stream2, b->ev_front, 0));
+    HIP_TRY(hipEventRecord(b->ev_lane_go, c.stream));
+    HIP_TRY(hipStreamWaitEvent(b->stream2, b->ev_lane_go, 0));
     if (f16 && (rc = BeginRange(b->exec2, b->stream2))) return rc;
   }
   const Operand op{c.d_yt, b->d_y2, c.ldy, ZeroSource(c), b->d_shift4};
-  const Lane lanes[2] = {{c.stream, &c.exec}, {b->stream2, &b->exec2}};
+  const Lane lanes[2] = {{c.stream, &c.exec, pipelined ? b->ev_consumed : nullptr}, {b->stream2, &b->exec2, pipelined ? b->ev_consumed2 : nullptr}};
   if ((rc = WalkChunks(am, op, b->total_rows, c.chunk, lanes, two ? 2 : 1, true, prob_scale, c.d_ll, tm))) return rc;
+  if (pipelined) { b->lay_dirty = false; b->consumed_new = true; }
   if (two) {
     if (f16 && (rc = CollectRange(b->exec2, b->stream2))) return rc;
     HIP_TRY(hipEventRecord(b->ev_lane2, b->stream2));
     HIP_TRY(hipStreamWaitEvent(c.stream, b->ev_lane2, 0));
   }
   if (f16) {
-    if ((rc = CollectRange(c.exec, c.stream))) return rc;
+    if ((rc = CollectRange(c.exec, c.stream, first_own))) return rc;
     b->range_pending = true;
     b->range_status = 0;
   }
@@ -726,6 +824,7 @@
 int pk_mi355_batch_synchronize(pk_mi355_batch_t *b) {
   if (!b) return Fail(PK_MI355_E_INVALID, "null batch");
   HIP_TRY(hipStreamSynchronize(b->core.stream));
+  if (b->in_dirty) HIP_TRY(hipStreamSynchronize(b->in_stream));
   return BatchRangeStatus(b);
 }
 
@@ -830,6 +929,7 @@
   const int T = b->h_T[utt];
   if (T == 0) return 0;
   const int D = b->core.am->feat_dim;
+  if (int rc = JoinInput(b)) return rc;
   HIP_TRY(hipMemcpyAsync(out, b->d_raw + b->h_raw_base[utt] * D, sizeof(float) * (size_t)T * D, hipMemcpyDeviceToHost, b->core.stream));
   HIP_TRY(hipStreamSynchronize(b->core.stream));
   return 0;
@@ -842,6 +942,7 @@
   if (T == 0) return 0;
   const int D = b->core.am->feat_dim;
   std::vector<float> tmp((size_t)D * T);
+  if (int rc = JoinInput(b)) return rc;
   HIP_TRY(hipMemcpy2DAsync(tmp.data(), sizeof(float) * T, b->core.d_yt + b->h_pad_base[utt] + b->core.am->left,
                            sizeof(float) * b->core.ldy, sizeof(float) * T, D, hipMemcpyDeviceToHost, b->core.stream));
   HIP_TRY(hipStreamSynchronize(b->core.stream));
diff --git a/pocketkaldi_amd/csrc/capi_exec.hip b/pocketkaldi_amd/csrc/capi_exec.hip
--- a/pocketkaldi_amd/csrc/capi_exec.hip
+++ b/pocketkaldi_amd/csrc/capi_exec.hip
@@ -60,12 +60,14 @@
   *e = ExecBufs();
 }
 
-int BeginRange(const ExecBufs &e, hipStream_t s) {
-  if (e.range) HIP_TRY(hipMemsetAsync(e.range, 0, sizeof(uint32_t) * e.range_words, s));
-  return 0;
-}
-int CollectRange(const ExecBufs &e, hipStream_t s) {
-  if (e.range) HIP_TRY(hipMemcpyAsync(e.h_range, e.range, sizeof(uint32_t) * e.range_words, hipMemcpyDeviceToHost, s));
+int BeginRange(const ExecBufs &e, hipStream_t s, int l0, int l1) {
+  const int w0 = std::min(l0 * kRangeSlots, e.range_words), w1 = std::min<int64_t>((int64_t)l1 * kRangeSlots, e.range_words);
+  if (e.range && w1 > w0) HIP_TRY(hipMemsetAsync(e.range + w0, 0, sizeof(uint32_t) * (w1 - w0), s));
+  return 0;
+}
+int CollectRange(const ExecBufs &e, hipStream_t s, int l0, int l1) {
+  const int w0 = std::min(l0 * kRangeSlots, e.range_words), w1 = std::min<int64_t>((int64_t)l1 * kRangeSlots, e.range_words);
+  if (e.range && w1 > w0) HIP_TRY(hipMemcpyAsync(e.h_range + w0, e.range + w0, sizeof(uint32_t) * (w1 - w0), hipMemcpyDeviceToHost, s));
   return 0;
 }
 void ClearHostRange(const ExecBufs &e) {
@@ -101,7 +103,7 @@
 int RunLayers(const pk_mi355_am *am, const ExecBufs &e, const float *q0, int64_t ldq,
               int splice_dim, int rows, bool want_tail, float scale, float *tail_out,
               int64_t tail_ld, hipStream_t stream, Timer *timer, ExecResult *res, const float *splice_zero = nullptr,
-              const int32_t *splice_shift = nullptr) {
+              const int32_t *splice_shift = nullptr, hipEvent_t consumed = nullptr) {
   const int rows_pad = (int)RoundUp(rows, kTile);
   if (splice_dim > 0 && !splice_zero) return Fail(PK_MI355_E_INVALID, "spliced input without a zero source");
   if (rows_pad > e.rows_cap) return Fail(PK_MI355_E_INVALID, "chunk larger than workspace");
@@ -192,6 +194,7 @@
           }
           LaunchGemm(g, stream);
         }
+        if (cur_splice && consumed) HIP_TRY(hipEventRecord(consumed, stream));
         cur = dst; cur_ld = g.ldo; cur_rows = rows_out; cur_splice = false; cur_dim = D.N;
         next_buf ^= 1;
         if (fuse_relu) ++i;
@@ -264,7 +267,8 @@
 
 int RunLayersF16(const pk_mi355_am *am, const ExecBufs &e, const _Float16 *x, int64_t ldx, int rows,
                  bool want_tail, float scale, float *tail_out,
-                 int64_t tail_ld, hipStream_t stream, Timer *timer, ExecResult *res, const int32_t *row_shift4 = nullptr) {
+                 int64_t tail_ld, hipStream_t stream, Timer *timer, ExecResult *res, const int32_t *row_shift4 = nullptr,
+                 hipEvent_t consumed = nullptr) {
   const int rows_pad = (int)RoundUp(rows, kTileF16);
   if (rows_pad > e.rows_cap) return Fail(PK_MI355_E_INVALID, "chunk larger than workspace");
   const float *blob = am->d_blob;
@@ -300,6 +304,7 @@
       Scoped t(timer, PK_MI355_K_GEMM, stream);
       LaunchGemmF16(g, stream);
     }
+    if (li == 0 && consumed) HIP_TRY(hipEventRecord(consumed, stream));
     if (norm) {
       Scoped t(timer, PK_MI355_K_OTHER, stream);
       LaunchNormalizeSplitF16(e.a, D.Npad, rows_pad, D.N, D.Npad, e.h[buf], 2 * D.Npad, ExpX(am, li + 1), RangeOf(e, li + 1), stream);
@@ -336,8 +341,9 @@
     const Lane &l = lanes[r0 / chunk % nlanes];
     const int32_t *shift4 = op.shift4 ? op.shift4 + r0 / 4 : nullptr;
     float *dst = out + r0 * N;
-    const int rc = f16 ? RunLayersF16(am, *l.exec, op.y2 + r0 * 2 * D, 2 * D, rows, want_tail, scale, dst, N, l.stream, timer, nullptr, shift4)
-                       : RunLayers(am, *l.exec, op.yt + r0, op.ld, D, rows, want_tail, scale, dst, N, l.stream, timer, nullptr, op.zero, shift4);
+    const hipEvent_t consumed = r0 + nlanes * chunk >= total_rows ? l.consumed : nullptr;
+    const int rc = f16 ? RunLayersF16(am, *l.exec, op.y2 + r0 * 2 * D, 2 * D, rows, want_tail, scale, dst, N, l.stream, timer, nullptr, shift4, consumed)
+                       : RunLayers(am, *l.exec, op.yt + r0, op.ld, D, rows, want_tail, scale, dst, N, l.stream, timer, nullptr, op.zero, shift4, consumed);
     if (rc) return rc;
   }
   return 0;
diff --git a/pocketkaldi_amd/csrc/pk_host.h b/pocketkaldi_amd/csrc/pk_host.h
--- a/pocketkaldi_amd/csrc/pk_host.h
+++ b/pocketkaldi_amd/csrc/pk_host.h
@@ -153,8 +153,8 @@
 constexpr float kRangeSaturated = 65504.0f;
 constexpr float kRangeTooSmall = 0.03125f;
 
-int BeginRange(const ExecBufs &e, hipStream_t s);
-int CollectRange(const ExecBufs &e, hipStream_t s);
+int BeginRange(const ExecBufs &e, hipStream_t s, int l0 = 0, int l1 = 1 << 20);
+int CollectRange(const ExecBufs &e, hipStream_t s, int l0 = 0, int l1 = 1 << 20);
 void ClearHostRange(const ExecBufs &e);
 int EvalRange(const pk_mi355_am *am, const ExecBufs *const *bufs, int nbufs);
 void FreeWorkspace(Workspace *w);
diff --git a/pocketkaldi_amd/csrc/pk_score.h b/pocketkaldi_amd/csrc/pk_score.h
--- a/pocketkaldi_amd/csrc/pk_score.h
+++ b/pocketkaldi_amd/csrc/pk_score.h
@@ -74,7 +74,7 @@
 bool ExpandShift4(const std::vector<ShiftSpan> &spans, int64_t total_rows, int64_t zero_span, int32_t *shift4, int32_t *bad);
 
 struct Operand { const float *yt; const _Float16 *y2; int64_t ld; const float *zero; const int32_t *shift4; };
-struct Lane { hipStream_t stream; const ExecBufs *exec; };
+struct Lane { hipStream_t stream; const ExecBufs *exec; hipEvent_t consumed = nullptr; };
 int WalkChunks(const pk_mi355_am *am, const Operand &op, int64_t total_rows, int64_t chunk, const Lane *lanes, int nlanes,
                bool want_tail, float scale, float *out, Timer *timer);
 
```
